# dotchen/LearningByCheating

Hardware: AMD Instinct MI355X
Metric: images/sec ImagePolicyModelSS phase-1 train @ bs256 (higher is better)
Workload: dtype bf16; 1 GPU; ImagePolicyModelSS(resnet34) phase-1 step vs BirdViewPolicyModelSS(resnet18) teacher [phase1_bs256_bf16], 160x384 RGB + 7x192x192 bird-view uint8 NHWC frames as the dataset stores them (2048-frame dataset per rank resident in HBM, a different batch every step), global batch 256 (256/GPU), bf16 MFMA operands and bf16 activation storage + f32 accumulate/master weights/gradients/BN/loss/Adam, local B; global_batch=256, parallelism=dp1

## Files before the change

### learningbycheating_amd/csrc/c_api_ops.cpp

```cpp
#include "lbc_common.hpp"
#include "lbc_hip.h"
#include "lbc_kernels.hpp"
#include <string.h>
#include <algorithm>

namespace {
size_t up64(size_t n) { return (n + 63) / 64 * 64; }
NormConst imagenet(int enabled)
{
    NormConst nc;
    memset(&nc, 0, sizeof(nc));
    nc.enabled = enabled;
    const float m3[3] = {0.485f, 0.456f, 0.406f}, s3[3] = {0.229f, 0.224f, 0.225f};
    for (int i = 0; i < 3; ++i) { nc.mean[i] = m3[i]; nc.stdv[i] = s3[i]; }
    return nc;
}
#define LBC_TRY(expr)            \
    do {                         \
        int rc__ = (expr);       \
        if (rc__) return rc__;   \
    } while (0)
}

extern "C" {

int lbc_bn_stats(const void* x, long long pixels, int C, int act_bf16, float* partial, int* rows, lbc_stream_t stream)
{
    LBC_REQUIRE(pixels > 0 && C > 0 && C % 8 == 0 && C / 4 <= 256, "bn_stats: bad shape (%lld pixels, C = %d)", pixels, C);
    if (rows) *rows = lbc_chan_reduce_rows(pixels, C);
    if (!x) return LBC_OK;
    LBC_REQUIRE(partial, "bn_stats: null partial buffer");
    ChanReduceArgs r;
    memset(&r, 0, sizeof(r));
    r.x = x; r.partial = partial; r.pixels = pixels; r.C = C; r.act_bf16 = act_bf16;
    return lbc_chan_reduce(r, 0, (hipStream_t)stream);
}

int lbc_bn_finalize_stats(const float* partial, int rows, int C, long long count, const float* gamma, const float* beta,
                          float* running_mean, float* running_var, long long* num_batches_tracked, float momentum, float eps,
                          int train, float* scale, float* shift, float* save_mean, float* save_invstd, lbc_stream_t stream)
{
    LBC_REQUIRE(scale && shift && C > 0, "bn_finalize_stats: null output");
    LBC_REQUIRE(!train || (partial && rows >= 1 && rows <= kLbcFinalizeRows && count > 0), "bn_finalize_stats: training mode needs 1..%d partial rows",
                kLbcFinalizeRows);
    LBC_REQUIRE(train || (running_mean && running_var), "bn_finalize_stats: eval mode needs the running statistics");
    LBC_REQUIRE((running_mean == nullptr) == (running_var == nullptr) && (save_mean == nullptr) == (save_invstd == nullptr),
                "bn_finalize_stats: running_mean/var and save_mean/invstd come in pairs");
    BnFinalizeArgs f;
    memset(&f, 0, sizeof(f));
    f.partial = partial; f.rows = rows; f.C = C; f.count = count; f.gamma = gamma; f.beta = beta;
    f.running_mean = running_mean; f.running_var = running_var; f.num_batches_tracked = num_batches_tracked;
    f.momentum = momentum; f.eps = eps; f.train = train;
    f.scale = scale; f.shift = shift; f.save_mean = save_mean; f.save_invstd = save_invstd;
    return lbc_bn_finalize(f, (hipStream_t)stream);
}

int lbc_bn_apply_relu_add_fwd(const void* x, void* y, long long pixels, int C, const float* scale, const float* shift,
                              const void* resid, const float* rscale, const float* rshift, int relu, int act_bf16,
                              lbc_stream_t stream)
{
    LBC_REQUIRE(x && y && scale && shift, "bn_apply: null argument");
    LBC_REQUIRE((rscale == nullptr) == (rshift == nullptr) && (!rscale || resid), "bn_apply: residual affine without a residual");
    BnApplyArgs a;
    memset(&a, 0, sizeof(a));
    a.x = x; a.y = y; a.pixels = pixels; a.C = C; a.scale = scale; a.shift = shift;
    a.resid = resid; a.rscale = rscale; a.rshift = rshift; a.relu = relu; a.act_bf16 = act_bf16;
    return lbc_bn_apply(a, (hipStream_t)stream);
}

size_t lbc_bn_bwd_workspace(int C) { return (up64((size_t)kLbcFinalizeRows * 2 * C) + 3 * up64((size_t)C)) * sizeof(float); }

int lbc_bn_bwd(const void* x, const void* dz, const void* mask, const float* mask_scale, const float* mask_shift,
               void* g_out, const float* gamma, const float* mean, const float* invstd, long long pixels, int C, int Cout,
               float* dgamma, float* dbeta, void* dx, float* workspace, int act_bf16, lbc_stream_t stream)
{
    LBC_REQUIRE(x && dz && mean && invstd && dx && workspace, "bn_bwd: null argument");
    LBC_REQUIRE(pixels > 0 && C % 8 == 0 && C / 4 <= 256 && Cout % 8 == 0 && Cout <= C, "bn_bwd: bad shape");
    LBC_REQUIRE(g_out || !mask_scale, "bn_bwd: an affine mask needs g_out (the apply pass reads the stored masked gradient)");
    hipStream_t s = (hipStream_t)stream;
    float* partial = workspace;
    float* cA = partial + up64((size_t)kLbcFinalizeRows * 2 * C);
    float* cB = cA + up64((size_t)C);
    float* cD = cB + up64((size_t)C);
    ChanReduceArgs r;
    memset(&r, 0, sizeof(r));
    r.x = x; r.dz = dz; r.mask = mask; r.mask_scale = mask_scale; r.mask_shift = mask_shift; r.g_out = g_out;
    r.mean = mean; r.invstd = invstd; r.partial = partial; r.pixels = pixels; r.C = C; r.act_bf16 = act_bf16;
    LBC_TRY(lbc_chan_reduce(r, 1, s));
    const int rows = lbc_chan_reduce_rows(pixels, C);
    BnBwdFinalizeArgs f;
    memset(&f, 0, sizeof(f));
    f.partial = partial; f.rows = rows; f.C = C; f.count = pixels; f.gamma = gamma; f.mean = mean; f.invstd = invstd; f.train = 1;
    f.dgamma = dgamma; f.dbeta = dbeta; f.coefA = cA; f.coefB = cB; f.coefD = cD;
    LBC_TRY(lbc_bn_bwd_finalize(f, s));
    BnBwdApplyArgs ap;
    memset(&ap, 0, sizeof(ap));
    ap.g = g_out ? g_out : dz; ap.mask = g_out ? nullptr : mask; ap.x = x;
    ap.coefA = cA; ap.coefB = cB; ap.coefD = cD; ap.mean = mean; ap.invstd = invstd;
    ap.dx = dx; ap.pixels = pixels; ap.C = C; ap.Cout = Cout; ap.act_bf16 = act_bf16;
    return lbc_bn_bwd_apply(ap, s);
}

int lbc_maxpool3x3s2_fwd(const void* y, const float* scale, const float* shift, void* p, unsigned char* idx, int N, int H, int W,
                         int C, int act_bf16, lbc_stream_t stream)
{
    LBC_REQUIRE(y && scale && shift && p && N > 0, "maxpool_fwd: null argument");
    PoolFwdArgs a;
    memset(&a, 0, sizeof(a));
    a.y = y; a.scale = scale; a.shift = shift; a.p = p; a.idx = idx; a.N = N; a.H = H; a.W = W; a.C = C; a.act_bf16 = act_bf16;
    return lbc_bn_relu_maxpool_fwd(a, (hipStream_t)stream);
}

int lbc_maxpool3x3s2_bwd(const void* dp, const unsigned char* idx, const void* y, const float* scale, const float* shift,
                         const float* mean, const float* invstd, void* g, float* partial, int* rows, int N, int H, int W, int C,
                         int act_bf16, lbc_stream_t stream)
{
    LBC_REQUIRE(N > 0 && H > 0 && W > 0 && C % 8 == 0 && C / 4 <= 256, "maxpool_bwd: bad shape");
    if (rows) *rows = lbc_pool_bwd_rows(N, H, W, C);
    if (!dp) return LBC_OK;
    LBC_REQUIRE(idx && y && scale && shift && mean && invstd && g && partial, "maxpool_bwd: null argument");
    PoolBwdArgs a;
    memset(&a, 0, sizeof(a));
    a.dp = dp; a.idx = idx; a.y = y; a.scale = scale; a.shift = shift; a.mean = mean; a.invstd = invstd; a.g = g; a.partial = partial;
    a.N = N; a.H = H; a.W = W; a.C = C; a.act_bf16 = act_bf16;
    return lbc_maxpool_relu_bwd_reduce(a, (hipStream_t)stream);
}

namespace {
struct HeadWs { float* rowstat; float* s_partial; float* partial2; float* coef; float* scratch; };
HeadWs head_ws(float* w, int N)
{
    HeadWs h;
    h.rowstat = w;
    h.s_partial = h.rowstat + up64((size_t)N * 40);
    h.partial2 = h.s_partial + up64((size_t)lbc_head_bwd_max_rows(N) * 20 * 65);
    h.coef = h.partial2 + up64((size_t)8 * 20 * 65);
    h.scratch = h.coef + up64((size_t)3 * 64);
    return h;
}
void head_args(const lbc_head_desc* d, HeadArgs& ha)
{
    memset(&ha, 0, sizeof(ha));
    ha.h = d->h; ha.act_bf16 = d->act_bf16; ha.N = d->N; ha.OH = d->OH; ha.OW = d->OW; ha.cmd = d->cmd;
    for (int b = 0; b < 4; ++b) {
        ha.mean[b] = d->mean[b]; ha.invstd[b] = d->invstd[b]; ha.gamma[b] = d->gamma[b]; ha.beta[b] = d->beta[b];
        ha.w[b] = d->w[b]; ha.bias[b] = d->bias[b]; ha.pos_x[b] = d->pos_x[b]; ha.pos_y[b] = d->pos_y[b];
    }
}
}

size_t lbc_head_workspace(int N)
{
    if (N < 1) return 0;
    return (up64((size_t)N * 40) + up64((size_t)lbc_head_bwd_max_rows(N) * 20 * 65) + up64((size_t)8 * 20 * 65) + up64((size_t)3 * 64) +
            up64((size_t)N * 16 * 20 * 4)) * sizeof(float);
}

int lbc_head_fwd(const lbc_head_desc* d, float* pred_all, float* pred_sel, float* workspace, lbc_stream_t stream)
{
    LBC_REQUIRE(d && d->h && d->cmd && pred_all && workspace, "head_fwd: null argument");
    HeadArgs ha;
    head_args(d, ha);
    const HeadWs ws = head_ws(workspace, d->N);
    ha.pred_all = pred_all; ha.pred_sel = pred_sel; ha.rowstat = ws.rowstat; ha.scratch = ws.scratch;
    return lbc_head_fwd(ha, (hipStream_t)stream);
}

int lbc_head_bwd(const lbc_head_desc* d, const float* pred_all, const float* d_all, const float* d_sel, void* dh,
                 float* const* dgamma, float* const* dbeta, float* const* dw, float* const* dbias, float* workspace,
                 lbc_stream_t stream)
{
    LBC_REQUIRE(d && d->h && d->cmd && pred_all && dh && dgamma && dbeta && dw && dbias && workspace, "head_bwd: null argument");
    hipStream_t s = (hipStream_t)stream;
    const int N = d->N;
    const HeadWs ws = head_ws(workspace, N);
    HeadBwdArgs hb;
    memset(&hb, 0, sizeof(hb));
    head_args(d, hb.f);
    hb.f.pred_all = const_cast<float*>(pred_all); hb.f.rowstat = ws.rowstat;
    hb.d_all = d_all; hb.d_sel = d_sel; hb.s_partial = ws.s_partial; hb.dh = dh; hb.chan_coef = ws.coef;
    LBC_TRY(lbc_head_bwd_reduce(hb, s));
    HeadBwdFinalizeArgs hf;
    memset(&hf, 0, sizeof(hf));
    hf.s_partial = ws.s_partial; hf.rows = lbc_head_bwd_rows(hb.f); hf.count = (long long)N * d->OH * d->OW;
    if (hf.rows > 8) {
        LBC_TRY(lbc_partial_reduce(ws.s_partial, hf.rows, 20 * 65, ws.partial2, 8, s));
        hf.s_partial = ws.partial2; hf.rows = 8;
    }
    for (int b = 0; b < 4; ++b) {
        hf.gamma[b] = d->gamma[b]; hf.beta[b] = d->beta[b]; hf.w[b] = d->w[b];
        hf.dgamma[b] = dgamma[b]; hf.dbeta[b] = dbeta[b]; hf.dw[b] = dw[b]; hf.dbias[b] = dbias[b];
    }
    hf.mean = d->mean[0]; hf.invstd = d->invstd[0]; hf.chan_coef = ws.coef;
    LBC_TRY(lbc_head_bwd_finalize(hf, s));
    return lbc_head_bwd_apply(hb, s);
}

int lbc_nchw_to_input(const float* image_nchw, void* xp, int xp_bf16, int N, int C, int H, int W, int normalize, lbc_stream_t stream)
{
    LBC_REQUIRE(image_nchw && xp && N > 0 && (!normalize || C == 3), "nchw_to_input: bad arguments");
    return lbc_prep_input(image_nchw, xp, xp_bf16, N, C, H, W, imagenet(normalize), (hipStream_t)stream);
}

int lbc_u8nhwc_to_input(const unsigned char* image_nhwc, void* xp, int xp_bf16, int N, int C, int H, int W, int normalize,
                        lbc_stream_t stream)
{
    LBC_REQUIRE(image_nhwc && xp && N > 0 && (!normalize || C == 3), "u8nhwc_to_input: bad arguments");
    return lbc_prep_input_u8(image_nhwc, xp, xp_bf16, N, C, H, W, imagenet(normalize), (hipStream_t)stream);
}

int lbc_stem_fwd(const void* xp, const float* w, void* y, float* stats, int* stats_rows, int N, int H, int W, int C, int bf16,
                 lbc_stream_t stream)
{
    LBC_REQUIRE(N > 0 && bf16 >= 0 && bf16 <= 2, "stem_fwd: bad arguments");
    StemArgs st;
    memset(&st, 0, sizeof(st));
    st.xp = xp; st.xp_bf16 = bf16 != 0; st.w = w; st.y = y; st.stats = stats;
    st.N = N; st.H = H; st.W = W; st.Cin = C; st.act_bf16 = bf16 == 2; st.bf16 = bf16 != 0;
    if (stats_rows) *stats_rows = lbc_stem_rows(st);
    if (!y) return LBC_OK;
    LBC_REQUIRE(xp && w, "stem_fwd: null argument");
    return lbc_stem_fwd(st, (hipStream_t)stream);
}

size_t lbc_stem_wgrad_workspace(int N, int H, int W, int C)
{
    const int ns = std::max(lbc_stem_wgrad_split(N, H, W, C, 0), lbc_stem_wgrad_split(N, H, W, C, 1));
    return (size_t)ns * 64 * 49 * C * sizeof(float);
}

int lbc_stem_wgrad(const void* xp, const void* dy, float* dw, void* workspace, int N, int H, int W, int C, int bf16,
                   lbc_stream_t stream)
{
    LBC_REQUIRE(xp && dy && dw && workspace && N > 0 && bf16 >= 0 && bf16 <= 2, "stem_wgrad: bad arguments");
    StemWgradArgs sw;
    memset(&sw, 0, sizeof(sw));
    sw.xp = xp; sw.xp_bf16 = bf16 != 0; sw.dy = dy; sw.partial = static_cast<float*>(workspace);
    sw.N = N; sw.H = H; sw.W = W; sw.Cin = C; sw.act_bf16 = bf16 == 2; sw.bf16 = bf16 != 0;
    sw.nsplit = lbc_stem_wgrad_split(N, H, W, C, bf16 != 0);
    LBC_TRY(lbc_stem_wgrad(sw, (hipStream_t)stream));
    return lbc_splitk_reduce(sw.partial, sw.nsplit, (long long)64 * 49 * C, dw, 0.f, (hipStream_t)stream);
}

int lbc_birdview_crop_u8(const unsigned char* src, unsigned char* dst, int N, int SH, int SW, int C, int y0, int x0, int H, int W,
                         lbc_stream_t stream)
{
    return lbc_crop_u8(src, dst, N, SH, SW, C, y0, x0, H, W, (hipStream_t)stream);
}

int lbc_birdview_warp_crop_u8(const unsigned char* src, unsigned char* dst, const lbc_warp_params* params_dev, int N, int SH, int SW, int C,
                              int H, int W, lbc_stream_t stream)
{
    static_assert(sizeof(lbc_warp_params) == sizeof(WarpParams), "warp parameter layout");
    return lbc_warp_crop_u8(src, dst, reinterpret_cast<const WarpParams*>(params_dev), N, SH, SW, C, H, W, (hipStream_t)stream);
}

int lbc_augment_rgb_u8(unsigned char* images, const lbc_aug_params* params_dev, float* scratch, int N, int H, int W, int any_blur,
                       lbc_stream_t stream)
{
    static_assert(sizeof(lbc_aug_params) == sizeof(AugParams), "augmentation parameter layout");
    return lbc_augment_u8(images, reinterpret_cast<const AugParams*>(params_dev), scratch, N, H, W, any_blur, (hipStream_t)stream);
}

int lbc_replay_cdf(const float* w, int n, double* cdf, long long* bad_count, lbc_stream_t stream)
{
    return lbc_replay_cdf_launch(w, n, cdf, bad_count, (hipStream_t)stream);
}

int lbc_replay_sample(const double* cdf, int n, unsigned seed, unsigned long long step, int B, int* idx, lbc_stream_t stream)
{
    return lbc_replay_sample_launch(cdf, n, seed, step, B, idx, (hipStream_t)stream);
}

int lbc_replay_gather_u8(const unsigned char* src, long long row_bytes, const int* idx, int B, int reps, unsigned char* dst, lbc_stream_t stream)
{
    return lbc_replay_gather_launch(src, row_bytes, idx, B, reps, dst, (hipStream_t)stream);
}

int lbc_replay_scatter_u8(const unsigned char* src, long long row_bytes, const int* slot, int M, unsigned char* dst, lbc_stream_t stream)
{
    return lbc_replay_scatter_launch(src, row_bytes, slot, M, dst, (hipStream_t)stream);
}

int lbc_replay_meta(const float* speed, const int* cmd, const int* idx, int B, int reps, float* speed_out, float* onehot_out, lbc_stream_t stream)
{
    return lbc_replay_meta_launch(speed, cmd, idx, B, reps, speed_out, onehot_out, (hipStream_t)stream);
}

int lbc_replay_writeback(const float* w_batch, const int* idx, int B, int reps, int n, float* new_w, lbc_stream_t stream)
{
    return lbc_replay_writeback_launch(w_batch, idx, B, reps, n, new_w, (hipStream_t)stream);
}

}
```

### learningbycheating_amd/csrc/engine.cpp

```cpp
#include "engine.hpp"

#include <algorithm>
#include <stdlib.h>
#include <string.h>

namespace lbc {

namespace {
constexpr float kBnMomentum = 0.1f;
constexpr float kBnEps = 1e-5f;
size_t up64(size_t n) { return (n + 63) / 64 * 64; }
#define LBC_TRY(expr)            \
    do {                         \
        int rc__ = (expr);       \
        if (rc__) return rc__;   \
    } while (0)
}

int Net::add_tensor(const std::string& name, int kind, std::initializer_list<int> shape)
{
    TensorInfo ti;
    ti.name = name;
    ti.kind = kind;
    ti.ndim = (int)shape.size();
    ti.numel = 1;
    int i = 0;
    for (int s : shape) { ti.shape[i++] = s; ti.numel *= s; }
    for (; i < 4; ++i) ti.shape[i] = 1;
    t_.push_back(ti);
    return (int)t_.size() - 1;
}

size_t Net::alloc(size_t nfloats)
{
    const size_t off = ws_floats_;
    ws_floats_ += up64(nfloats);
    return off;
}

size_t Net::alloc_act(size_t n) { return alloc(act_bf16_ ? (n + 1) / 2 : n); }

BN Net::make_bn(const std::string& p, int C)
{
    BN bn;
    bn.C = C;
    bn.g = add_tensor(p + ".weight", kParam, {C});
    bn.b = add_tensor(p + ".bias", kParam, {C});
    bn.rm = add_tensor(p + ".running_mean", kBufferF32, {C});
    bn.rv = add_tensor(p + ".running_var", kBufferF32, {C});
    bn.nbt = add_tensor(p + ".num_batches_tracked", kBufferI64, {});
    bn.scale = alloc(C); bn.shift = alloc(C); bn.mean = alloc(C); bn.invstd = alloc(C);
    bn.cA = alloc(C); bn.cB = alloc(C); bn.cD = alloc(C);
    return bn;
}

Conv Net::make_conv(const std::string& name, int Cin, int Cout, int H, int W, int k, int s, int p)
{
    Conv c;
    c.w = add_tensor(name, kParam, {Cout, Cin, k, k});
    c.Cin = Cin; c.Cout = Cout; c.H = H; c.W = W; c.k = k; c.s = s; c.p = p;
    c.OH = (H + 2 * p - k) / s + 1;
    c.OW = (W + 2 * p - k) / s + 1;
    c.y = alloc_act((size_t)d_.max_batch * c.OH * c.OW * Cout);
    if (act_bf16_) { c.wn = alloc(((size_t)Cout * Cin * k * k + 1) / 2); c.wt = alloc(((size_t)Cout * Cin * k * k + 1) / 2); }
    return c;
}

Net::Net(const lbc_net_desc& d) : d_(d)
{
    const size_t NB = (size_t)d.max_batch;
    const int Cin = d.in_channels, H0 = d.H, W0 = d.W;
    side_allowed_ = !lbc_opt_on(kOptNoSideStream);
    bf16_ = d.precision >= 1;
    act_bf16_ = d.precision == 2;
    x3_ = d.precision == 3;
    stem_bf16_ = bf16_ && !x3_;
    defer_wgrad_ = act_bf16_;
    if (defer_wgrad_) side_allowed_ = false;
    if (bf16_) dgrad_wt_ = true;

    stem_w_ = add_tensor("conv.conv1.weight", kParam, {64, Cin, 7, 7});
    stem_bn_ = make_bn("conv.bn1", 64);
    xp_ = alloc(NB * (H0 + 6) * (W0 + 6) * Cin);
    y0_ = alloc_act(NB * (H0 / 2) * (W0 / 2) * 64);
    H1_ = H0 / 4; W1_ = W0 / 4;
    p0_ = alloc_act(NB * H1_ * W1_ * 64);
    idx_ = alloc(NB * H1_ * W1_ * 64 / 4);

    const int n34[4] = {3, 4, 6, 3}, n18[4] = {2, 2, 2, 2};
    const int* nb = d.arch == 34 ? n34 : n18;
    int inpl = 64, h = H1_, w = W1_;
    size_t max_act = NB * H1_ * W1_ * 64;
    for (int li = 0; li < 4; ++li) {
        const int planes = 64 << li;
        stage_first_block_.push_back((int)blocks_.size());
        for (int bi = 0; bi < nb[li]; ++bi) {
            const int stride = (li > 0 && bi == 0) ? 2 : 1;
            const std::string pre = "conv.layer" + std::to_string(li + 1) + "." + std::to_string(bi);
            Block b;
            b.c1 = make_conv(pre + ".conv1.weight", inpl, planes, h, w, 3, stride, 1);
            b.b1 = make_bn(pre + ".bn1", planes);
            const int oh = b.c1.OH, ow = b.c1.OW;
            b.c2 = make_conv(pre + ".conv2.weight", planes, planes, oh, ow, 3, 1, 1);
            b.b2 = make_bn(pre + ".bn2", planes);
            if (stride != 1 || inpl != planes) {
                b.has_ds = true;
                b.ds = make_conv(pre + ".downsample.0.weight", inpl, planes, h, w, 1, stride, 0);
                b.bd = make_bn(pre + ".downsample.1", planes);
            }
            b.fuse_z1 = planes == 64 || !conv_takes_glds(b.c2, (int)NB) || conv_takes_glds(b.c2, (int)NB, true);
            b.z1 = b.fuse_z1 ? 0 : alloc_act(NB * oh * ow * planes);
            b.out = alloc_act(NB * oh * ow * planes);
            blocks_.push_back(b);
            inpl = planes; h = oh; w = ow;
        }
    }

    hcat_ = alloc_act(NB * h * w * 640);
    const int dc[4] = {640, 256, 128, 64};
    const char* bn_name[3] = {"deconv.0", "deconv.3", "deconv.6"};
    const char* ct_name[3] = {"deconv.1", "deconv.4", "deconv.7"};
    int dh = h, dw = w;
    for (int i = 0; i < 3; ++i) {
        Deconv& D = dec_[i];
        D.bn = make_bn(bn_name[i], dc[i]);
        D.w = add_tensor(std::string(ct_name[i]) + ".weight", kParam, {dc[i], dc[i + 1], 3, 3});
        D.bias = add_tensor(std::string(ct_name[i]) + ".bias", kParam, {dc[i + 1]});
        D.Cin = dc[i]; D.Cout = dc[i + 1]; D.H = dh; D.W = dw;
        D.u = alloc_act(NB * (2 * dh) * (2 * dw) * dc[i + 1]);
        if (act_bf16_) { D.wn = alloc(((size_t)dc[i] * dc[i + 1] * 9 + 1) / 2); D.wt = alloc(((size_t)dc[i] * dc[i + 1] * 9 + 1) / 2); }
        dh *= 2; dw *= 2;
        max_act = std::max(max_act, NB * dh * dw * (size_t)dc[i + 1]);
    }
    HH_ = dh; HW_ = dw;

    for (int b = 0; b < 4; ++b) {
        const std::string pre = "location_pred." + std::to_string(b);
        head_bn_[b] = make_bn(pre + ".0", 64);
        head_w_[b] = add_tensor(pre + ".1.weight", kParam, {5, 64, 1, 1});
        head_b_[b] = add_tensor(pre + ".1.bias", kParam, {5});
        head_px_[b] = add_tensor(pre + ".2.pos_x", kBufferF32, {HH_ * HW_});
        head_py_[b] = add_tensor(pre + ".2.pos_y", kBufferF32, {HH_ * HW_});
    }
    head_stats_ = alloc(2 * 64);
    head_coef_ = alloc(3 * 64);
    head_partial_ = alloc(std::max((size_t)lbc_head_bwd_max_rows((int)NB) * 20 * 65, NB * 16 * 20 * 4));
    pred_all_ = alloc(NB * 40);
    rowstat_ = alloc(NB * 40);
    cmd_ = alloc(NB * 4);

    size_t pf = 1024 * 2 * 640;
    pf = std::max(pf, (size_t)lbc_cdiv((long long)NB * (H0 / 2) * (W0 / 2), 128) * 128);
    for (const Block& b : blocks_) {
        pf = std::max(pf, (size_t)lbc_cdiv((long long)NB * b.c1.OH * b.c1.OW, 64) * 2 * b.c1.Cout);
    }
    for (int i = 0; i < 3; ++i)
        pf = std::max(pf, (size_t)4 * lbc_cdiv((long long)NB * dec_[i].H * dec_[i].W, 64) * 2 * dec_[i].Cout);
    partial_floats_ = pf;
    partial_ = alloc(pf);
    partial2_floats_ = (size_t)64 * 2 * 640;
    partial2_ = alloc(partial2_floats_);

    size_t wg = 0;
    auto wg_need = [&](int N, int OH, int OW, int CP, int Hq, int Wq, int CQ, int k, int s, int p) {
        WgradArgs a;
        memset(&a, 0, sizeof(a));
        a.N = N; a.OH = OH; a.OW = OW; a.CP = CP; a.H = Hq; a.W = Wq; a.CQ = CQ; a.KH = k; a.KW = k; a.S = s; a.P = p;
        a.bf16 = bf16_; a.act_bf16 = act_bf16_; a.x3 = x3_;
        return (size_t)lbc_wgrad_pick_split(a) * CP * k * k * CQ;
    };
    for (const Block& b : blocks_) {
        wg = std::max(wg, wg_need((int)NB, b.c1.OH, b.c1.OW, b.c1.Cout, b.c1.H, b.c1.W, b.c1.Cin, 3, b.c1.s, 1));
        wg = std::max(wg, wg_need((int)NB, b.c2.OH, b.c2.OW, b.c2.Cout, b.c2.H, b.c2.W, b.c2.Cin, 3, 1, 1));
        if (b.has_ds) wg = std::max(wg, wg_need((int)NB, b.ds.OH, b.ds.OW, b.ds.Cout, b.ds.H, b.ds.W, b.ds.Cin, 1, b.ds.s, 0));
    }
    for (int i = 0; i < 3; ++i)
        wg = std::max(wg, wg_need((int)NB, dec_[i].H, dec_[i].W, dec_[i].Cin, 2 * dec_[i].H, 2 * dec_[i].W, dec_[i].Cout, 3, 2, 1));
    wg = std::max(wg, (size_t)lbc_stem_wgrad_split((int)NB, H0, W0, Cin, stem_bf16_) * 64 * 49 * Cin);
    if (defer_wgrad_) {
        for (size_t li = 0; li < stage_first_block_.size(); ++li) {
            const size_t first = stage_first_block_[li], last = li + 1 < stage_first_block_.size() ? (size_t)stage_first_block_[li + 1] : blocks_.size();
            size_t members = 0, dy = 0;
            for (size_t bi = first; bi < last; ++bi) {
                const Block& b = blocks_[bi];
                const size_t slot = (((size_t)NB * b.c1.OH * b.c1.OW * b.c1.Cout + 1) / 2 + 63) / 64 * 64;
                members += 1 + (b.c1.s == 1 ? 1 : 0);
                dy += (b.has_ds ? 3 : 2) * slot;
            }
            const Conv& c = blocks_[last - 1].c2;
            WgradArgs a;
            memset(&a, 0, sizeof(a));
            a.N = (int)NB; a.OH = c.OH; a.OW = c.OW; a.CP = c.Cout; a.H = c.H; a.W = c.W; a.CQ = c.Cin; a.KH = 3; a.KW = 3; a.S = 1; a.P = 1;
            a.bf16 = 1; a.act_bf16 = 1; a.p = &a; a.q = &a;
            if (lbc_wgrad_tr_eligible(a)) {
                for (int n = 1; n <= (int)std::min(members, (size_t)kLbcWgradGroupMax); ++n)
                    wg = std::max(wg, (size_t)lbc_wgrad_tr_group_split(a, n) * n * c.Cout * 9 * c.Cin);
            }
            dy_arena_floats_ = std::max(dy_arena_floats_, dy);
        }
        dy_arena_ = alloc(dy_arena_floats_);
    }
    wg_partial_ = alloc(wg);
    wg_floats_ = wg;

    wt_ = alloc((size_t)640 * 512 * 9);
    gD_ = alloc_act(max_act); gE_ = alloc_act(max_act); gF_ = alloc_act(max_act); gG_ = alloc_act(max_act);
    g0_ = alloc_act(NB * (H0 / 2) * (W0 / 2) * 64);
}

std::vector<Net::ActInfo> Net::activations() const
{
    std::vector<ActInfo> v;
    const int ae = act_bf16_ ? 2 : 4;
    auto add = [&](const std::string& name, size_t off_floats, int H, int W, int C, int elem) {
        v.push_back(ActInfo{name, off_floats * sizeof(float), H, W, C, elem});
    };
    add("conv.conv1", y0_, d_.H / 2, d_.W / 2, 64, ae);
    add("conv.maxpool", p0_, H1_, W1_, 64, ae);
    add("conv.maxpool.idx", idx_, H1_, W1_, 64, 1);
    int li = 0;
    for (size_t i = 0; i < blocks_.size(); ++i) {
        while (li + 1 < (int)stage_first_block_.size() && (int)i >= stage_first_block_[li + 1]) ++li;
        const Block& b = blocks_[i];
        const std::string p = "conv.layer" + std::to_string(li + 1) + "." + std::to_string((int)i - stage_first_block_[li]);
        add(p + ".conv1", b.c1.y, b.c1.OH, b.c1.OW, b.c1.Cout, ae);
        add(p + ".bn1.scale", b.b1.scale, 1, 1, b.b1.C, 4);
        add(p + ".bn1.shift", b.b1.shift, 1, 1, b.b1.C, 4);
        add(p + ".conv2", b.c2.y, b.c2.OH, b.c2.OW, b.c2.Cout, ae);
        if (b.has_ds) add(p + ".downsample.0", b.ds.y, b.ds.OH, b.ds.OW, b.ds.Cout, ae);
        add(p, b.out, b.c2.OH, b.c2.OW, b.c2.Cout, ae);
    }
    for (int i = 0; i < 3; ++i) add("deconv." + std::to_string(3 * i + 2), dec_[i].u, 2 * dec_[i].H, 2 * dec_[i].W, dec_[i].Cout, ae);
    return v;
}

Net::~Net()
{
    if (side_) (void)hipStreamDestroy(side_);
    if (ev_fork_) (void)hipEventDestroy(ev_fork_);
    if (ev_join_) (void)hipEventDestroy(ev_join_);
}

int Net::fork(hipStream_t s)
{
    if (!side_on_) return LBC_OK;
    if (hipEventRecord(ev_fork_, s) != hipSuccess || hipStreamWaitEvent(side_, ev_fork_, 0) != hipSuccess) {
        lbc_set_error("net.backward: side-stream fork failed");
        return LBC_ELAUNCH;
    }
    side_dirty_ = true;
    return LBC_OK;
}

int Net::join(hipStream_t s)
{
    if (!side_on_ || !side_dirty_) return LBC_OK;
    if (hipEventRecord(ev_join_, side_) != hipSuccess || hipStreamWaitEvent(s, ev_join_, 0) != hipSuccess) {
        lbc_set_error("net.backward: side-stream join failed");
        return LBC_ELAUNCH;
    }
    side_dirty_ = false;
    return LBC_OK;
}

int Net::check_bound(bool need_grads) const
{
    if (!ws_) { lbc_set_error("net: workspace not bound"); return LBC_ESTATE; }
    for (const TensorInfo& t : t_) {
        if (!t.ptr) { lbc_set_error("net: tensor %s not bound", t.name.c_str()); return LBC_ESTATE; }
        if (need_grads && t.kind == kParam && !t.grad) { lbc_set_error("net: gradient of %s not bound", t.name.c_str()); return LBC_ESTATE; }
    }
    return LBC_OK;
}

int Net::conv_fwd(const Conv& c, const float* x, int N, bool stats, int* rows, hipStream_t s, const BN* pre, const BN* post,
                  const float* resid, bool relu, float* out, float* stats_buf, size_t stats_cap)
{
    IgemmArgs a;
    memset(&a, 0, sizeof(a));
    a.x = x; a.w = P(c.w); a.y = out ? out : W(c.y);
    if (pre) { a.pre_scale = W(pre->scale); a.pre_shift = W(pre->shift); a.pre_relu = 1; }
    if (post) { a.post_scale = W(post->scale); a.post_shift = W(post->shift); }
    a.resid = resid; a.relu = relu ? 1 : 0;
    a.N = N; a.H = c.H; a.W = c.W; a.C = c.Cin;
    a.OH = c.OH; a.OW = c.OW; a.K = c.Cout;
    a.KH = c.k; a.KW = c.k; a.S = c.s; a.P = c.p;
    a.M = N * c.OH * c.OW; a.LH = c.OH; a.LW = c.OW; a.ostep = 1;
    a.bf16 = bf16_; a.act_bf16 = act_bf16_; a.x3 = x3_;
    if (act_bf16_) { a.w = W(c.wn); a.w_bf16 = 1; }
    split_scratch(a);
    const int cfg = lbc_igemm_pick_for(a, 0);
    *rows = lbc_igemm_rows(a, cfg);
    a.stats = stats ? (stats_buf ? stats_buf : W(partial_)) : nullptr;
    LBC_REQUIRE(!a.stats || (size_t)*rows * 2 * (size_t)c.Cout <= (stats_buf ? stats_cap : partial_floats_),
                "net: %d statistics rows of %d channels exceed their buffer", *rows, c.Cout);
    return lbc_igemm_launch(a, 1, 0, cfg, s);
}

void Net::split_scratch(IgemmArgs& a) const
{
    if (!defer_wgrad_ || side_on_ || !wg_floats_) return;
    a.split_ws = W(wg_partial_);
    a.split_ws_floats = (long long)wg_floats_;
}

bool Net::conv_takes_glds(const Conv& c, int N, bool with_prologue) const
{
    if (!act_bf16_) return false;
    IgemmArgs a;
    memset(&a, 0, sizeof(a));
    a.N = N; a.H = c.H; a.W = c.W; a.C = c.Cin; a.OH = c.OH; a.OW = c.OW; a.K = c.Cout;
    a.KH = c.k; a.KW = c.k; a.S = c.s; a.P = c.p; a.M = N * c.OH * c.OW; a.LH = c.OH; a.LW = c.OW; a.ostep = 1;
    a.bf16 = 1; a.act_bf16 = 1; a.w_bf16 = 1;
    if (with_prologue) { a.pre_scale = reinterpret_cast<const float*>(this); a.pre_shift = a.pre_scale; a.pre_relu = 1; }
    return lbc_igemm_pick_for(a, 0) >= kLbcCfgGlds;
}

int Net::weight_prep(hipStream_t s)
{
    WeightPrepArgs a;
    memset(&a, 0, sizeof(a));
    int n = 0, tiles = 0;
    auto add = [&](const float* w, size_t wn, size_t wt, int A, int T, int B) {
        if (n >= WeightPrepArgs::kMax) return false;
        WeightPrepItem& it = a.item[n++];
        it.w = w; it.wn = W(wn); it.wt = W(wt); it.A = A; it.T = T; it.B = B; it.tile_begin = tiles;
        tiles += lbc_weight_prep_tiles(A, T, B);
        return true;
    };
    bool ok = true;
    for (const Block& b : blocks_) {
        ok = ok && add(P(b.c1.w), b.c1.wn, b.c1.wt, b.c1.Cout, 9, b.c1.Cin);
        ok = ok && add(P(b.c2.w), b.c2.wn, b.c2.wt, b.c2.Cout, 9, b.c2.Cin);
        if (b.has_ds) ok = ok && add(P(b.ds.w), b.ds.wn, b.ds.wt, b.ds.Cout, 1, b.ds.Cin);
    }
    for (int i = 0; i < 3; ++i) ok = ok && add(P(dec_[i].w), dec_[i].wn, dec_[i].wt, dec_[i].Cin, 9, dec_[i].Cout);
    LBC_REQUIRE(ok, "net: more than %d convolution weights", WeightPrepArgs::kMax);
    a.count = n; a.tiles = tiles;
    return lbc_weight_prep(a, s);
}

int Net::bn_eval_prep(hipStream_t s)
{
    BnEvalArgs a;
    memset(&a, 0, sizeof(a));
    int n = 0;
    bool ok = true;
    auto add = [&](const BN& bn) {
        if (n >= BnEvalArgs::kMax) { ok = false; return; }
        BnEvalItem& it = a.item[n++];
        it.gamma = P(bn.g); it.beta = P(bn.b); it.running_mean = P(bn.rm); it.running_var = P(bn.rv);
        it.scale = W(bn.scale); it.shift = W(bn.shift); it.mean = W(bn.mean); it.invstd = W(bn.invstd);
        it.C = bn.C;
    };
    add(stem_bn_);
    for (const Block& b : blocks_) { add(b.b1); add(b.b2); if (b.has_ds) add(b.bd); }
    for (int i = 0; i < 3; ++i) add(dec_[i].bn);
    for (int b = 0; b < 4; ++b) add(head_bn_[b]);
    LBC_REQUIRE(ok, "net: more than %d BatchNorms", BnEvalArgs::kMax);
    a.count = n; a.eps = kBnEps;
    return lbc_bn_eval_prep(a, s);
}

int Net::set_sync_bn(lbc_allreduce_fn fn, void* ctx, int world, float* buf, int buf_floats)
{
    if (!fn) { sync_fn_ = nullptr; sync_ctx_ = nullptr; sync_world_ = 1; sync_buf_ = nullptr; return LBC_OK; }
    LBC_REQUIRE(world >= 1 && buf && buf_floats >= kSyncFloats, "net.set_sync_bn: world_size >= 1 and a buffer of >= %d floats",
                kSyncFloats);
    sync_fn_ = fn; sync_ctx_ = ctx; sync_world_ = world; sync_buf_ = buf;
    return LBC_OK;
}

int Net::sync_rows(const float*& part, int& rows, int width, int n_local, hipStream_t s, float* local_lo, float* local_hi)
{
    if (!sync_fn_) return LBC_OK;
    LBC_REQUIRE(width + 1 <= kSyncFloats, "net: %d sums do not fit the SyncBN buffer", width);
    if (rows > kLbcFinalizeRows) {
        LBC_TRY(lbc_partial_reduce(part, rows, width, W(partial2_), 64, s));
        part = W(partial2_); rows = 64;
    }
    LBC_TRY(lbc_partial_reduce(part, rows, width, sync_buf_, 1, s, local_lo, local_hi, (float)n_local));
    if (sync_fn_(sync_ctx_, sync_buf_, width + 1, s) != 0) {
        lbc_set_error("net: the SyncBN all-reduce callback failed");
        return LBC_ELAUNCH;
    }
    part = sync_buf_; rows = 1;
    return LBC_OK;
}

int Net::bn_finalize(const BN& bn, int rows, long long count, int n_local, int train, hipStream_t s, bool update_running, const float* synced)
{
    const float* part = W(partial_);
    const float* nsum = nullptr;
    if (train && synced) {
        part = synced; rows = 1; nsum = synced + 2 * bn.C;
    } else if (train && sync_fn_) {
        LBC_TRY(sync_rows(part, rows, 2 * bn.C, n_local, s));
        nsum = part + 2 * bn.C;
    } else if (train && rows > kLbcFinalizeRows) {
        LBC_TRY(lbc_partial_reduce(W(partial_), rows, 2 * bn.C, W(partial2_), 64, s));
        part = W(partial2_);
        rows = 64;
    }
    BnFinalizeArgs f = fin_args(bn, part, rows, count, update_running);
    f.nsum = nsum; f.n_local = n_local; f.train = train;
    if (!train) { f.running_mean = P(bn.rm); f.running_var = P(bn.rv); f.num_batches_tracked = nullptr; }
    return lbc_bn_finalize(f, s);
}

BnFinalizeArgs Net::fin_args(const BN& bn, const float* part, int rows, long long count, bool update_running) const
{
    BnFinalizeArgs f;
    memset(&f, 0, sizeof(f));
    f.partial = part; f.rows = rows; f.C = bn.C; f.count = count;
    f.gamma = P(bn.g); f.beta = P(bn.b);
    f.running_mean = update_running ? P(bn.rm) : nullptr;
    f.running_var = update_running ? P(bn.rv) : nullptr;
    f.num_batches_tracked = update_running ? static_cast<long long*>(t_[bn.nbt].ptr) : nullptr;
    f.momentum = kBnMomentum; f.eps = kBnEps; f.train = 1;
    f.scale = W(bn.scale); f.shift = W(bn.shift); f.save_mean = W(bn.mean); f.save_invstd = W(bn.invstd);
    return f;
}

int Net::forward(int N, int train, const void* image, int image_u8, const float* velocity, const float* command, float* pred_sel,
                 float* pred_all, hipStream_t s)
{
    LBC_REQUIRE(N >= 1 && N <= d_.max_batch, "net.forward: batch %d outside [1,%d]", N, d_.max_batch);
    LBC_REQUIRE(image && velocity && command && pred_all, "net.forward: null argument");
    LBC_TRY(check_bound(false));
    lastN_ = N; last_train_ = train; ++generation_;
    const int H0 = d_.H, W0 = d_.W, Cin = d_.in_channels;
    const bool tr = train != 0;
    int rows = 0;

    LBC_TRY(lbc_copy_f32(command, W(cmd_), 4 * N, s));
    NormConst nc;
    memset(&nc, 0, sizeof(nc));
    nc.enabled = d_.normalize;
    const float m3[3] = {0.485f, 0.456f, 0.406f}, s3[3] = {0.229f, 0.224f, 0.225f};
    for (int i = 0; i < 3; ++i) { nc.mean[i] = m3[i]; nc.stdv[i] = s3[i]; }
    if (image_u8) LBC_TRY(lbc_prep_input_u8(static_cast<const unsigned char*>(image), W(xp_), stem_bf16_, N, Cin, H0, W0, nc, s));
    else          LBC_TRY(lbc_prep_input(static_cast<const float*>(image), W(xp_), stem_bf16_, N, Cin, H0, W0, nc, s));
    const bool reuse = frozen_ && derived_valid_ && !tr;
    if (act_bf16_ && !reuse) LBC_TRY(weight_prep(s));
    if (!tr && !reuse) LBC_TRY(bn_eval_prep(s));
    derived_valid_ = frozen_ && !tr;

    StemArgs st;
    st.xp = W(xp_); st.xp_bf16 = stem_bf16_; st.w = P(stem_w_); st.y = W(y0_); st.stats = tr ? W(partial_) : nullptr;
    st.N = N; st.H = H0; st.W = W0; st.Cin = Cin; st.act_bf16 = act_bf16_; st.bf16 = stem_bf16_;
    LBC_TRY(lbc_stem_fwd(st, s));
    if (tr) LBC_TRY(bn_finalize(stem_bn_, lbc_stem_rows(st), (long long)N * (H0 / 2) * (W0 / 2), N, train, s));
    PoolFwdArgs pf;
    pf.y = W(y0_); pf.scale = W(stem_bn_.scale); pf.shift = W(stem_bn_.shift); pf.p = W(p0_);
    pf.idx = reinterpret_cast<unsigned char*>(W(idx_));
    pf.N = N; pf.H = H0 / 2; pf.W = W0 / 2; pf.C = 64; pf.act_bf16 = act_bf16_;
    LBC_TRY(lbc_bn_relu_maxpool_fwd(pf, s));

    const float* x = W(p0_);
    for (Block& b : blocks_) {
        const long long pix = (long long)N * b.c1.OH * b.c1.OW;
        if (!tr) {
            LBC_TRY(conv_fwd(b.c1, x, N, false, &rows, s, nullptr, &b.b1, nullptr, true));
            const float* identity = x;
            if (b.has_ds) {
                LBC_TRY(conv_fwd(b.ds, x, N, false, &rows, s, nullptr, &b.bd, nullptr, false));
                identity = W(b.ds.y);
            }
            LBC_TRY(conv_fwd(b.c2, W(b.c1.y), N, false, &rows, s, nullptr, &b.b2, identity, true, W(b.out)));
            x = W(b.out);
            continue;
        }
        LBC_TRY(conv_fwd(b.c1, x, N, tr, &rows, s));
        const bool fold1 = !b.fuse_z1 && can_fold(rows, b.b1.C);
        if (!fold1) LBC_TRY(bn_finalize(b.b1, rows, pix, N, train, s));
        BnApplyArgs ap;
        if (b.fuse_z1) {
            LBC_TRY(conv_fwd(b.c2, W(b.c1.y), N, tr, &rows, s, &b.b1));
        } else {
            memset(&ap, 0, sizeof(ap));
            ap.x = W(b.c1.y); ap.y = W(b.z1); ap.pixels = pix; ap.C = b.c1.Cout;
            ap.scale = W(b.b1.scale); ap.shift = W(b.b1.shift); ap.relu = 1; ap.act_bf16 = act_bf16_;
            if (fold1) { ap.fold = 1; ap.fin = fin_args(b.b1, W(partial_), rows, pix); }
            LBC_TRY(lbc_bn_apply(ap, s));
            LBC_TRY(conv_fwd(b.c2, W(b.z1), N, tr, &rows, s));
        }
        const bool fold2 = can_fold(rows, b.b2.C) && (!b.has_ds || (size_t)lbc_cdiv(pix, 64) * 2 * b.bd.C <= partial2_floats_);
        const int rows2 = rows;
        if (!fold2) LBC_TRY(bn_finalize(b.b2, rows, pix, N, train, s));
        memset(&ap, 0, sizeof(ap));
        ap.x = W(b.c2.y); ap.y = W(b.out); ap.pixels = pix; ap.C = b.c2.Cout;
        ap.scale = W(b.b2.scale); ap.shift = W(b.b2.shift); ap.relu = 1; ap.act_bf16 = act_bf16_;
        if (fold2) { ap.fold = 1; ap.fin = fin_args(b.b2, W(partial_), rows2, pix); }
        if (b.has_ds) {
            float* dsp = fold2 ? W(partial2_) : W(partial_);
            LBC_TRY(conv_fwd(b.ds, x, N, tr, &rows, s, nullptr, nullptr, nullptr, false, nullptr, dsp, fold2 ? partial2_floats_ : partial_floats_));
            if (fold2 && can_fold(rows, b.bd.C)) { ap.rfold = 1; ap.rfin = fin_args(b.bd, dsp, rows, pix); }
            else if (fold2) LBC_TRY(lbc_bn_finalize(fin_args(b.bd, dsp, rows, pix), s));
            else LBC_TRY(bn_finalize(b.bd, rows, pix, N, train, s));
            ap.resid = W(b.ds.y); ap.rscale = W(b.bd.scale); ap.rshift = W(b.bd.shift);
        } else {
            ap.resid = x;
        }
        LBC_TRY(lbc_bn_apply(ap, s));
        x = W(b.out);
    }

    const Block& last = blocks_.back();
    const int th = last.c2.OH, tw = last.c2.OW;
    LBC_TRY(lbc_concat_velocity(x, velocity, W(hcat_), N, th * tw, 512, 128, act_bf16_, s));
    if (tr) {
        ChanReduceArgs cr;
        memset(&cr, 0, sizeof(cr));
        cr.x = W(hcat_); cr.partial = W(partial_); cr.pixels = (long long)N * th * tw; cr.C = 640; cr.act_bf16 = act_bf16_;
        cr.max_rows = fold_rows_for(cr.pixels, 640);
        LBC_TRY(lbc_chan_reduce(cr, 0, s));
        rows = lbc_chan_reduce_rows(cr.pixels, 640, cr.max_rows);
    }
    int pend_rows = rows;
    long long pend_count = (long long)N * th * tw;
    const float* din = W(hcat_);
    for (int i = 0; i < 3; ++i) {
        Deconv& D = dec_[i];
        IgemmArgs a;
        memset(&a, 0, sizeof(a));
        a.x = din; a.w = P(D.w); a.y = W(D.u); a.bias = P(D.bias); a.relu = 1;
        a.pre_scale = W(D.bn.scale); a.pre_shift = W(D.bn.shift);
        a.N = N; a.H = D.H; a.W = D.W; a.C = D.Cin;
        a.OH = 2 * D.H; a.OW = 2 * D.W; a.K = D.Cout;
        a.KH = 3; a.KW = 3; a.S = 2; a.P = 1;
        a.LH = D.H; a.LW = D.W; a.ostep = 2;
        a.M = N * D.H * D.W;
        a.stats = tr ? W(partial_) : nullptr;
        a.act_bf16 = act_bf16_;
        int wmajor = 0;
        if (act_bf16_) {
            a.w = W(D.wt); a.w_bf16 = 1; a.bf16 = 1; wmajor = 1;
        } else if (bf16_) {
            LBC_TRY(lbc_weight_transpose(P(D.w), W(wt_), D.Cin, 9, D.Cout, s));
            a.w = W(wt_); a.bf16 = 1; a.x3 = x3_; wmajor = 1;
        }
        a.nphase = 4;
        int cfg = lbc_igemm_pick(a.M, a.K);
        if (act_bf16_) {
            IgemmArgs b = a;
            b.pre_scale = nullptr; b.pre_shift = nullptr; b.x = W(gF_);
            const int c2 = lbc_igemm_pick_for(b, 1);
            if (c2 >= kLbcCfgGlds) {
                BnApplyArgs ap;
                memset(&ap, 0, sizeof(ap));
                ap.x = din; ap.y = W(gF_); ap.pixels = (long long)N * D.H * D.W; ap.C = D.Cin;
                ap.scale = W(D.bn.scale); ap.shift = W(D.bn.shift); ap.relu = 0; ap.act_bf16 = 1;
                if (tr && can_fold(pend_rows, D.Cin)) { ap.fold = 1; ap.fin = fin_args(D.bn, W(partial_), pend_rows, pend_count); pend_rows = 0; }
                else if (tr) { LBC_TRY(bn_finalize(D.bn, pend_rows, pend_count, N, train, s)); pend_rows = 0; }
                LBC_TRY(lbc_bn_apply(ap, s));
                a = b; cfg = c2;
            }
        }
        if (tr && pend_rows > 0) LBC_TRY(bn_finalize(D.bn, pend_rows, pend_count, N, train, s));
        const int per = lbc_igemm_rows(a, cfg);
        LBC_TRY(lbc_igemm_launch(a, wmajor, 1, cfg, s));
        const long long opix = (long long)N * 4 * D.H * D.W;
        if (!tr) {
        } else if (i < 2) {
            pend_rows = 4 * per; pend_count = opix;
        } else {
            const float* part = W(partial_);
            int prow = 4 * per;
            LBC_TRY(sync_rows(part, prow, 2 * 64, N, s));
            {
                BnFinalizeArgs f = fin_args(head_bn_[0], part, prow, opix);
                if (sync_fn_) { f.nsum = part + 2 * 64; f.n_local = N; }
                else if (prow > kLbcFinalizeRows) {
                    LBC_TRY(lbc_partial_reduce(W(partial_), prow, 2 * 64, W(partial2_), 64, s));
                    f.partial = W(partial2_); f.rows = 64;
                }
                for (int b = 1; b < 4; ++b) {
                    f.more_running_mean[b - 1] = P(head_bn_[b].rm); f.more_running_var[b - 1] = P(head_bn_[b].rv);
                    f.more_num_batches_tracked[b - 1] = static_cast<long long*>(t_[head_bn_[b].nbt].ptr);
                }
                LBC_TRY(lbc_bn_finalize(f, s));
            }
        }
        din = W(D.u);
    }

    HeadArgs ha;
    memset(&ha, 0, sizeof(ha));
    ha.h = W(dec_[2].u);
    for (int b = 0; b < 4; ++b) {
        ha.mean[b] = W(head_bn_[tr ? 0 : b].mean);
        ha.invstd[b] = W(head_bn_[tr ? 0 : b].invstd);
        ha.gamma[b] = P(head_bn_[b].g); ha.beta[b] = P(head_bn_[b].b);
        ha.w[b] = P(head_w_[b]); ha.bias[b] = P(head_b_[b]);
        ha.pos_x[b] = P(head_px_[b]); ha.pos_y[b] = P(head_py_[b]);
    }
    ha.cmd = W(cmd_);
    ha.pred_all = W(pred_all_); ha.pred_sel = pred_sel; ha.rowstat = W(rowstat_);
    ha.N = N; ha.OH = HH_; ha.OW = HW_; ha.act_bf16 = act_bf16_;
    ha.scratch = W(head_partial_);
    LBC_TRY(lbc_head_fwd(ha, s));
    return lbc_copy_f32(W(pred_all_), pred_all, 40 * N, s);
}

int Net::bn_bwd_finalize(BnBwdFinalizeArgs f, hipStream_t s)
{
    if (sync_fn_) {
        LBC_TRY(sync_rows(f.partial, f.rows, 2 * f.C, lastN_, s, f.dbeta, f.dgamma));
        f.nsum = f.partial + 2 * f.C; f.n_local = lastN_;
        f.dgamma = nullptr; f.dbeta = nullptr;
    }
    return lbc_bn_bwd_finalize(f, s);
}

int Net::bn_backward(const BN& bn, const float* dz, const float* mask, float* g_out, const float* x, long long pixels,
                     float* dx, int Cout, hipStream_t s, const BN* mask_bn, bool join_before_apply, int reduced_rows)
{
    int rows = reduced_rows;
    if (reduced_rows <= 0) {
        ChanReduceArgs r;
        memset(&r, 0, sizeof(r));
        r.x = x; r.dz = dz; r.mask = mask; r.g_out = g_out; r.mean = W(bn.mean); r.invstd = W(bn.invstd);
        if (mask_bn) { r.mask_scale = W(mask_bn->scale); r.mask_shift = W(mask_bn->shift); }
        r.partial = W(partial_); r.pixels = pixels; r.C = bn.C; r.act_bf16 = act_bf16_;
        r.max_rows = fold_rows_for(pixels, bn.C);
        LBC_TRY(lbc_chan_reduce(r, 1, s));
        rows = lbc_chan_reduce_rows(pixels, bn.C, r.max_rows);
    } else {
        mask = nullptr;
        g_out = const_cast<float*>(dz);
    }
    const float* part = W(partial_);
    if (rows > kLbcFinalizeRows) {
        LBC_TRY(lbc_partial_reduce(W(partial_), rows, 2 * bn.C, W(partial2_), 64, s));
        part = W(partial2_); rows = 64;
    }
    BnBwdFinalizeArgs f;
    memset(&f, 0, sizeof(f));
    f.partial = part; f.rows = rows; f.C = bn.C; f.count = pixels;
    f.gamma = P(bn.g); f.mean = W(bn.mean); f.invstd = W(bn.invstd); f.train = 1;
    f.dgamma = G(bn.g); f.dbeta = G(bn.b);
    f.coefA = W(bn.cA); f.coefB = W(bn.cB); f.coefD = W(bn.cD);
    const bool fold = can_fold(rows, bn.C) && (g_out || !mask);
    if (!fold) LBC_TRY(bn_bwd_finalize(f, s));
    BnBwdApplyArgs ap;
    memset(&ap, 0, sizeof(ap));
    if (fold) { ap.fold = 1; ap.fin = f; }
    ap.g = g_out ? g_out : dz; ap.mask = g_out ? nullptr : mask; ap.x = x;
    ap.coefA = W(bn.cA); ap.coefB = W(bn.cB); ap.coefD = W(bn.cD);
    ap.mean = W(bn.mean); ap.invstd = W(bn.invstd);
    ap.dx = dx; ap.pixels = pixels; ap.C = bn.C; ap.Cout = Cout; ap.act_bf16 = act_bf16_;
    if (join_before_apply) LBC_TRY(join(s));
    return lbc_bn_bwd_apply(ap, s);
}

float* Net::dy_slot(long long elems)
{
    const size_t floats = ((size_t)(elems + 1) / 2 + 63) / 64 * 64;
    if (dy_used_ + floats > dy_arena_floats_) return nullptr;
    float* p = W(dy_arena_) + dy_used_;
    dy_used_ += floats;
    return p;
}

int Net::flush_wgrads(int N, hipStream_t s)
{
    std::vector<char> done(pending_.size(), 0);
    for (size_t i = 0; i < pending_.size(); ++i) {
        if (done[i]) continue;
        const PendingWgrad& pi = pending_[i];
        const Conv& c = *pi.c;
        WgradArgs a;
        memset(&a, 0, sizeof(a));
        a.p = pi.dy; a.q = pi.x;
        if (pi.pre) { a.q_scale = W(pi.pre->scale); a.q_shift = W(pi.pre->shift); a.q_relu = 1; }
        a.bf16 = bf16_; a.act_bf16 = act_bf16_; a.x3 = x3_;
        a.N = N; a.OH = c.OH; a.OW = c.OW; a.CP = c.Cout; a.H = c.H; a.W = c.W; a.CQ = c.Cin;
        a.KH = c.k; a.KW = c.k; a.S = c.s; a.P = c.p;
        if (!lbc_wgrad_tr_eligible(a)) {
            LBC_TRY(conv_wgrad_pre(c, pi.x, pi.pre, pi.dy, N, s));
            done[i] = 1;
            continue;
        }
        WgradGroup g;
        memset(&g, 0, sizeof(g));
        float* grads[kLbcWgradGroupMax];
        for (size_t j = i; j < pending_.size() && g.n < kLbcWgradGroupMax; ++j) {
            const PendingWgrad& pj = pending_[j];
            const Conv& cj = *pj.c;
            if (done[j] || cj.Cout != c.Cout || cj.Cin != c.Cin || cj.H != c.H || cj.W != c.W || cj.k != c.k || cj.s != c.s || cj.p != c.p ||
                (pj.pre != nullptr) != (pi.pre != nullptr)) continue;
            g.p[g.n] = pj.dy; g.q[g.n] = pj.x;
            if (pj.pre) { g.q_scale[g.n] = W(pj.pre->scale); g.q_shift[g.n] = W(pj.pre->shift); }
            grads[g.n] = G(cj.w);
            ++g.n;
            done[j] = 1;
        }
        a.nsplit = lbc_wgrad_tr_group_split(a, g.n);
        const size_t count = (size_t)c.Cout * 9 * c.Cin;
        if ((size_t)a.nsplit * g.n * count > wg_floats_) a.nsplit = (int)std::max<size_t>(1, wg_floats_ / (g.n * count));
        for (int m = 0; m < g.n; ++m) g.out[m] = a.nsplit == 1 ? grads[m] : W(wg_partial_) + (size_t)m * a.nsplit * count;
        LBC_TRY(lbc_wgrad_tr_group_launch(a, g, s));
        if (a.nsplit > 1) LBC_TRY(lbc_splitk_reduce_group(W(wg_partial_), a.nsplit, (long long)count, g.n, grads, s));
    }
    pending_.clear();
    dy_used_ = 0;
    return LBC_OK;
}

int Net::conv_wgrad(const Conv& c, const float* x, const float* dy, int N, hipStream_t s)
{
    return conv_wgrad_pre(c, x, nullptr, dy, N, s);
}

int Net::conv_wgrad_pre(const Conv& c, const float* x, const BN* pre, const float* dy, int N, hipStream_t s)
{
    WgradArgs a;
    memset(&a, 0, sizeof(a));
    a.p = dy; a.q = x; a.partial = W(wg_partial_);
    if (pre) { a.q_scale = W(pre->scale); a.q_shift = W(pre->shift); a.q_relu = 1; }
    a.bf16 = bf16_; a.act_bf16 = act_bf16_; a.x3 = x3_;
    a.N = N; a.OH = c.OH; a.OW = c.OW; a.CP = c.Cout;
    a.H = c.H; a.W = c.W; a.CQ = c.Cin;
    a.KH = c.k; a.KW = c.k; a.S = c.s; a.P = c.p;
    a.nsplit = lbc_wgrad_pick_split(a);
    {
        const size_t count = (size_t)c.Cout * c.k * c.k * c.Cin;
        if ((size_t)a.nsplit * count > wg_floats_) a.nsplit = (int)std::max<size_t>(1, wg_floats_ / count);
    }
    if (a.nsplit == 1) { a.partial = G(c.w); return lbc_wgrad_launch(a, s); }
    LBC_TRY(lbc_wgrad_launch(a, s));
    return lbc_splitk_reduce(a.partial, a.nsplit, (long long)c.Cout * c.k * c.k * c.Cin, G(c.w), 0.f, s);
}

int Net::conv_dgrad(const Conv& c, const float* dy, const float* resid, float* dx, int N, hipStream_t s, const BN* bnb,
                    const float* bnb_y, int* fused_rows, const float* bnb_mask)
{
    if (fused_rows) *fused_rows = 0;
    IgemmArgs a;
    memset(&a, 0, sizeof(a));
    a.x = dy; a.w = P(c.w); a.y = dx; a.resid = resid;
    a.N = N; a.H = c.OH; a.W = c.OW; a.C = c.Cout;
    a.OH = c.H; a.OW = c.W; a.K = c.Cin;
    a.KH = c.k; a.KW = c.k; a.S = c.s; a.P = c.p;
    int wmajor = 0;
    a.bf16 = bf16_; a.act_bf16 = act_bf16_; a.x3 = x3_;
    if (act_bf16_) {
        a.w = W(c.wt); a.w_bf16 = 1; wmajor = 1;
    } else if (dgrad_wt_ && (c.k == 3 || bf16_)) {
        LBC_TRY(lbc_weight_transpose(P(c.w), W(wt_), c.Cout, c.k * c.k, c.Cin, s));
        a.w = W(wt_);
        wmajor = 1;
    }
    if (c.s == 1) {
        a.LH = c.H; a.LW = c.W; a.ostep = 1;
        a.M = N * c.H * c.W;
        split_scratch(a);
        const int cfg = wmajor ? lbc_igemm_pick_for(a, 1) : lbc_igemm_pick(a.M, a.K);
        if (bnb && bnb_y && fused_rows &&
            (bnb_mask ? lbc_igemm_fuses_bn_bwd_masked(a, wmajor, 1, cfg) : lbc_igemm_fuses_bn_bwd(a, wmajor, 1, cfg))) {
            a.bnb_y = bnb_y; a.bnb_scale = W(bnb->scale); a.bnb_shift = W(bnb->shift);
            a.bnb_mean = W(bnb->mean); a.bnb_invstd = W(bnb->invstd);
            a.bnb_mask = bnb_mask;
            a.stats = W(partial_);
            *fused_rows = lbc_igemm_rows(a, cfg);
            LBC_REQUIRE((size_t)*fused_rows * 2 * (size_t)a.K <= partial_floats_, "net: %d rows of BatchNorm-backward sums exceed their buffer", *fused_rows);
        }
        return lbc_igemm_launch(a, wmajor, 1, cfg, s);
    }
    a.LH = c.H / 2; a.LW = c.W / 2; a.ostep = 2;
    a.M = N * a.LH * a.LW;
    a.nphase = c.k == 1 ? 1 : 4;
    const int cfg = (wmajor && act_bf16_) ? lbc_igemm_pick_for(a, 1) : lbc_igemm_pick(a.M, a.K);
    return lbc_igemm_launch(a, wmajor, 1, cfg, s);
}

int Net::block_backward(Block& b, float*& D, float*& Gbuf, float* E, float* F, hipStream_t s)
{
    const int N = lastN_;
    const long long pix = (long long)N * b.c1.OH * b.c1.OW;
    const float* xin = (&b == &blocks_.front()) ? W(p0_) : W((&b - 1)->out);
    if (defer_wgrad_) {
        float* E2 = dy_slot(pix * b.b2.C);
        float* E1 = dy_slot(pix * b.b1.C);
        LBC_REQUIRE(E1 && E2, "net.backward: dY arena exhausted");
        const int pre_rows = bwd_pre_rows_;
        bwd_pre_rows_ = 0;
        LBC_REQUIRE(pre_rows == 0 || (bwd_pre_pix_ == pix && bwd_pre_C_ == b.b2.C), "net.backward: pre-reduced rows of %lld x %d do not match this block's bn2 (%lld x %d)",
                    bwd_pre_pix_, bwd_pre_C_, pix, b.b2.C);
        LBC_TRY(bn_backward(b.b2, D, W(b.out), D, W(b.c2.y), pix, E2, b.b2.C, s, nullptr, false, pre_rows));
        int fr = 0;
        LBC_TRY(conv_dgrad(b.c2, E2, nullptr, F, N, s, &b.b1, W(b.c1.y), &fr));
        if (b.fuse_z1) {
            pending_.push_back({&b.c2, W(b.c1.y), &b.b1, E2});
            LBC_TRY(bn_backward(b.b1, F, W(b.c1.y), F, W(b.c1.y), pix, E1, b.b1.C, s, &b.b1, false, fr));
        } else {
            pending_.push_back({&b.c2, W(b.z1), nullptr, E2});
            LBC_TRY(bn_backward(b.b1, F, W(b.z1), F, W(b.c1.y), pix, E1, b.b1.C, s, nullptr, false, fr));
        }
        pending_.push_back({&b.c1, xin, nullptr, E1});
        if (!b.has_ds) {
            Block* pb = (&b == &blocks_.front()) ? nullptr : (&b - 1);
            int pr = 0;
            if (pb) LBC_TRY(conv_dgrad(b.c1, E1, D, Gbuf, N, s, &pb->b2, W(pb->c2.y), &pr, W(pb->out)));
            else    LBC_TRY(conv_dgrad(b.c1, E1, D, Gbuf, N, s));
            bwd_pre_rows_ = pr;
            if (pr > 0) { bwd_pre_pix_ = (long long)N * pb->c2.OH * pb->c2.OW; bwd_pre_C_ = pb->b2.C; }
        } else {
            float* Fd = dy_slot(pix * b.bd.C);
            LBC_REQUIRE(Fd, "net.backward: dY arena exhausted");
            LBC_TRY(conv_dgrad(b.c1, E1, nullptr, Gbuf, N, s));
            LBC_TRY(bn_backward(b.bd, D, nullptr, nullptr, W(b.ds.y), pix, Fd, b.bd.C, s));
            pending_.push_back({&b.ds, xin, nullptr, Fd});
            LBC_TRY(conv_dgrad(b.ds, Fd, Gbuf, Gbuf, N, s));
        }
        std::swap(D, Gbuf);
        return LBC_OK;
    }
    LBC_TRY(bn_backward(b.b2, D, W(b.out), D, W(b.c2.y), pix, E, b.b2.C, s, nullptr, true));
    LBC_TRY(fork(s));
    int fr = 0;
    if (b.fuse_z1) {
        LBC_TRY(conv_wgrad_pre(b.c2, W(b.c1.y), &b.b1, E, N, wstream(s)));
        LBC_TRY(conv_dgrad(b.c2, E, nullptr, F, N, s, &b.b1, W(b.c1.y), &fr));
        LBC_TRY(bn_backward(b.b1, F, W(b.c1.y), F, W(b.c1.y), pix, E, b.b1.C, s, &b.b1, true, fr));
    } else {
        LBC_TRY(conv_wgrad(b.c2, W(b.z1), E, N, wstream(s)));
        LBC_TRY(conv_dgrad(b.c2, E, nullptr, F, N, s, &b.b1, W(b.c1.y), &fr));
        LBC_TRY(bn_backward(b.b1, F, W(b.z1), F, W(b.c1.y), pix, E, b.b1.C, s, nullptr, true, fr));
    }
    LBC_TRY(fork(s));
    LBC_TRY(conv_wgrad(b.c1, xin, E, N, wstream(s)));
    if (!b.has_ds) {
        LBC_TRY(conv_dgrad(b.c1, E, D, Gbuf, N, s));
    } else {
        LBC_TRY(conv_dgrad(b.c1, E, nullptr, Gbuf, N, s));
        LBC_TRY(bn_backward(b.bd, D, nullptr, nullptr, W(b.ds.y), pix, F, b.bd.C, s));
        LBC_TRY(fork(s));
        LBC_TRY(conv_wgrad(b.ds, xin, F, N, wstream(s)));
        LBC_TRY(conv_dgrad(b.ds, F, Gbuf, Gbuf, N, s));
    }
    std::swap(D, Gbuf);
    return LBC_OK;
}

int Net::backward(const float* d_sel, const float* d_all, int stage, hipStream_t s)
{
    const int rc = backward_impl(d_sel, d_all, stage, s);
    if (rc != LBC_OK) { pending_.clear(); dy_used_ = 0; bwd_pre_rows_ = 0; }
    if (rc != LBC_OK && side_dirty_) {
        (void)hipStreamSynchronize(side_);
        side_dirty_ = false;
    }
    return rc;
}

int Net::backward_impl(const float* d_sel, const float* d_all, int stage, hipStream_t s)
{
    LBC_REQUIRE(lastN_ > 0 && last_train_, "net.backward: needs a preceding training-mode forward");
    LBC_REQUIRE(stage >= -1 && stage < kNumStages, "net.backward: bad stage %d", stage);
    LBC_TRY(check_bound(true));
    const int N = lastN_;
    float* E = W(gE_);
    float* F = W(gF_);
    side_on_ = side_allowed_ && !lbc_prof_on();
    if (side_on_ && !side_) {
        int cur = 0, want = 0;
        (void)hipGetDevice(&cur);
        want = cur;
        hipPointerAttribute_t attr;
        if (hipPointerGetAttributes(&attr, ws_) == hipSuccess) want = attr.device;
        if (want != cur) (void)hipSetDevice(want);
        const bool ok = hipStreamCreateWithFlags(&side_, hipStreamNonBlocking) == hipSuccess &&
                        hipEventCreateWithFlags(&ev_fork_, hipEventDisableTiming) == hipSuccess &&
                        hipEventCreateWithFlags(&ev_join_, hipEventDisableTiming) == hipSuccess;
        if (want != cur) (void)hipSetDevice(cur);
        if (!ok) {
            lbc_set_error("net.backward: cannot create the side stream");
            return LBC_ELAUNCH;
        }
    }

    if (stage == -1 || stage == 0) {
        bwd_D_ = W(gD_); bwd_G_ = W(gG_);
        HeadBwdArgs hb;
        memset(&hb, 0, sizeof(hb));
        HeadArgs& ha = hb.f;
        ha.h = W(dec_[2].u);
        for (int b = 0; b < 4; ++b) {
            ha.mean[b] = W(head_bn_[0].mean); ha.invstd[b] = W(head_bn_[0].invstd);
            ha.gamma[b] = P(head_bn_[b].g); ha.beta[b] = P(head_bn_[b].b);
            ha.w[b] = P(head_w_[b]); ha.bias[b] = P(head_b_[b]);
            ha.pos_x[b] = P(head_px_[b]); ha.pos_y[b] = P(head_py_[b]);
        }
        ha.cmd = W(cmd_); ha.pred_all = W(pred_all_); ha.rowstat = W(rowstat_);
        ha.N = N; ha.OH = HH_; ha.OW = HW_; ha.act_bf16 = act_bf16_;
        hb.d_all = d_all; hb.d_sel = d_sel; hb.s_partial = W(head_partial_); hb.dh = E; hb.chan_coef = W(head_coef_);
        LBC_TRY(lbc_head_bwd_reduce(hb, s));
        HeadBwdFinalizeArgs hf;
        memset(&hf, 0, sizeof(hf));
        hf.s_partial = W(head_partial_); hf.rows = lbc_head_bwd_rows(hb.f); hf.count = (long long)N * HH_ * HW_;
        if (hf.rows > 8) {
            LBC_TRY(lbc_partial_reduce(W(head_partial_), hf.rows, 20 * 65, W(partial2_), 8, s));
            hf.s_partial = W(partial2_); hf.rows = 8;
        }
        for (int b = 0; b < 4; ++b) {
            hf.gamma[b] = P(head_bn_[b].g); hf.beta[b] = P(head_bn_[b].b); hf.w[b] = P(head_w_[b]);
            hf.dgamma[b] = G(head_bn_[b].g); hf.dbeta[b] = G(head_bn_[b].b);
            hf.dw[b] = G(head_w_[b]); hf.dbias[b] = G(head_b_[b]);
        }
        hf.mean = W(head_bn_[0].mean); hf.invstd = W(head_bn_[0].invstd); hf.chan_coef = W(head_coef_);
        LBC_TRY(lbc_head_bwd_finalize(hf, s));
        if (sync_fn_) {
            LBC_TRY(sync_rows(hf.s_partial, hf.rows, 20 * 65, N, s));
            hf.nsum = hf.s_partial + 20 * 65; hf.n_local = N; hf.coef_only = 1;
            LBC_TRY(lbc_head_bwd_finalize(hf, s));
        }
        LBC_TRY(lbc_head_bwd_apply(hb, s));

        for (int i = 2; i >= 0; --i) {
            Deconv& D = dec_[i];
            const float* xin = i == 0 ? W(hcat_) : W(dec_[i - 1].u);
            const long long opix = (long long)N * 4 * D.H * D.W;
            const long long ipix = (long long)N * D.H * D.W;
            ChanReduceArgs r;
            memset(&r, 0, sizeof(r));
            r.dz = E; r.mask = W(D.u); r.g_out = E; r.partial = W(partial_); r.pixels = opix; r.C = D.Cout; r.act_bf16 = act_bf16_;
            LBC_TRY(lbc_chan_reduce(r, 1, s));
            int rows = lbc_chan_reduce_rows(opix, D.Cout);
            const float* part = W(partial_);
            if (rows > kLbcFinalizeRows) {
                LBC_TRY(lbc_partial_reduce(W(partial_), rows, 2 * D.Cout, W(partial2_), 64, s));
                part = W(partial2_); rows = 64;
            }
            BnBwdFinalizeArgs f;
            memset(&f, 0, sizeof(f));
            f.partial = part; f.rows = rows; f.C = D.Cout; f.count = opix; f.dbeta = G(D.bias);
            LBC_TRY(lbc_bn_bwd_finalize(f, s));
            WgradArgs wa;
            memset(&wa, 0, sizeof(wa));
            wa.p = xin; wa.q = E; wa.partial = W(wg_partial_);
            wa.p_scale = W(D.bn.scale); wa.p_shift = W(D.bn.shift);
            wa.N = N; wa.OH = D.H; wa.OW = D.W; wa.CP = D.Cin;
            wa.H = 2 * D.H; wa.W = 2 * D.W; wa.CQ = D.Cout; wa.KH = 3; wa.KW = 3; wa.S = 2; wa.P = 1;
            wa.bf16 = bf16_; wa.act_bf16 = act_bf16_; wa.x3 = x3_;
            wa.nsplit = lbc_wgrad_pick_split(wa);
            if ((size_t)wa.nsplit * D.Cin * 9 * D.Cout > wg_floats_) wa.nsplit = (int)std::max<size_t>(1, wg_floats_ / ((size_t)D.Cin * 9 * D.Cout));
            if (wa.nsplit == 1) wa.partial = G(D.w);
            LBC_TRY(lbc_wgrad_launch(wa, s));
            if (wa.nsplit > 1) LBC_TRY(lbc_splitk_reduce(wa.partial, wa.nsplit, (long long)D.Cin * 9 * D.Cout, G(D.w), 0.f, s));
            IgemmArgs a;
            memset(&a, 0, sizeof(a));
            a.x = E; a.w = P(D.w); a.y = F;
            a.N = N; a.H = 2 * D.H; a.W = 2 * D.W; a.C = D.Cout;
            a.OH = D.H; a.OW = D.W; a.K = D.Cin; a.KH = 3; a.KW = 3; a.S = 2; a.P = 1;
            a.M = N * D.H * D.W; a.LH = D.H; a.LW = D.W; a.ostep = 1;
            a.bf16 = bf16_; a.act_bf16 = act_bf16_; a.x3 = x3_;
            if (act_bf16_) { a.w = W(D.wn); a.w_bf16 = 1; }
            LBC_TRY(lbc_igemm_launch(a, 1, 0, act_bf16_ ? lbc_igemm_pick_for(a, 0) : lbc_igemm_pick(a.M, a.K), s));
            float* dst = i == 0 ? bwd_D_ : E;
            LBC_TRY(bn_backward(D.bn, F, nullptr, nullptr, xin, ipix, dst, i == 0 ? 512 : D.Cin, s));
        }
    }

    for (int li = 3; li >= 0; --li) {
        const int st = 4 - li;
        if (stage != -1 && stage != st) continue;
        bwd_pre_rows_ = 0;
        const int first = stage_first_block_[li];
        const int lastb = li == 3 ? (int)blocks_.size() : stage_first_block_[li + 1];
        for (int bi = lastb - 1; bi >= first; --bi) LBC_TRY(block_backward(blocks_[bi], bwd_D_, bwd_G_, E, F, s));
        if (defer_wgrad_) LBC_TRY(flush_wgrads(N, s));
        LBC_TRY(join(s));
    }

    if (stage == -1 || stage == 5) {
        const int H0 = d_.H, W0 = d_.W;
        PoolBwdArgs pb;
        memset(&pb, 0, sizeof(pb));
        pb.dp = bwd_D_; pb.idx = reinterpret_cast<const unsigned char*>(W(idx_)); pb.y = W(y0_);
        pb.scale = W(stem_bn_.scale); pb.shift = W(stem_bn_.shift);
        pb.mean = W(stem_bn_.mean); pb.invstd = W(stem_bn_.invstd);
        pb.g = W(g0_); pb.partial = W(partial_);
        pb.N = N; pb.H = H0 / 2; pb.W = W0 / 2; pb.C = 64; pb.act_bf16 = act_bf16_;
        LBC_TRY(lbc_maxpool_relu_bwd_reduce(pb, s));
        int rows = lbc_pool_bwd_rows(N, H0 / 2, W0 / 2, 64);
        const long long pix = (long long)N * (H0 / 2) * (W0 / 2);
        const float* part = W(partial_);
        if (rows > kLbcFinalizeRows) {
            LBC_TRY(lbc_partial_reduce(W(partial_), rows, 128, W(partial2_), 64, s));
            part = W(partial2_); rows = 64;
        }
        BnBwdFinalizeArgs f;
        memset(&f, 0, sizeof(f));
        f.partial = part; f.rows = rows; f.C = 64; f.count = pix;
        f.gamma = P(stem_bn_.g); f.mean = W(stem_bn_.mean); f.invstd = W(stem_bn_.invstd); f.train = 1;
        f.dgamma = G(stem_bn_.g); f.dbeta = G(stem_bn_.b);
        f.coefA = W(stem_bn_.cA); f.coefB = W(stem_bn_.cB); f.coefD = W(stem_bn_.cD);
        LBC_TRY(bn_bwd_finalize(f, s));
        StemWgradArgs sw;
        memset(&sw, 0, sizeof(sw));
        if (lbc_stem_wgrad_fuses_bn_bwd(d_.in_channels, stem_bf16_)) {
            sw.bn_y = W(y0_); sw.bn_coefA = W(stem_bn_.cA); sw.bn_coefB = W(stem_bn_.cB); sw.bn_coefD = W(stem_bn_.cD);
            sw.bn_mean = W(stem_bn_.mean); sw.bn_invstd = W(stem_bn_.invstd);
        } else {
            BnBwdApplyArgs ap;
            memset(&ap, 0, sizeof(ap));
            ap.g = W(g0_); ap.x = W(y0_); ap.coefA = W(stem_bn_.cA); ap.coefB = W(stem_bn_.cB); ap.coefD = W(stem_bn_.cD);
            ap.mean = W(stem_bn_.mean); ap.invstd = W(stem_bn_.invstd);
            ap.dx = W(g0_); ap.pixels = pix; ap.C = 64; ap.Cout = 64; ap.act_bf16 = act_bf16_;
            LBC_TRY(lbc_bn_bwd_apply(ap, s));
        }
        sw.xp = W(xp_); sw.xp_bf16 = stem_bf16_; sw.dy = W(g0_); sw.partial = W(wg_partial_);
        sw.N = N; sw.H = H0; sw.W = W0; sw.Cin = d_.in_channels; sw.act_bf16 = act_bf16_; sw.bf16 = stem_bf16_;
        sw.nsplit = lbc_stem_wgrad_split(N, H0, W0, d_.in_channels, stem_bf16_);
        LBC_TRY(lbc_stem_wgrad(sw, s));
        LBC_TRY(lbc_splitk_reduce(sw.partial, sw.nsplit, (long long)64 * 49 * d_.in_channels, G(stem_w_), 0.f, s));
    }
    return LBC_OK;
}

}

struct lbc_net { lbc::Net impl; explicit lbc_net(const lbc_net_desc& d) : impl(d) {} };

extern "C" {

int lbc_net_create(const lbc_net_desc* d, lbc_net** out)
{
    LBC_REQUIRE(d && out, "net_create: null argument");
    LBC_REQUIRE(d->arch == 18 || d->arch == 34, "net_create: arch %d unsupported (BasicBlock ResNet-18/34 only)", d->arch);
    LBC_REQUIRE(d->in_channels == 3 || d->in_channels == 7, "net_create: in_channels %d unsupported", d->in_channels);
    LBC_REQUIRE(d->H > 0 && d->W > 0 && d->H % 32 == 0 && d->W % 32 == 0, "net_create: image %dx%d must be a multiple of 32", d->H, d->W);
    LBC_REQUIRE(d->max_batch >= 1, "net_create: max_batch %d", d->max_batch);
    LBC_REQUIRE(!d->normalize || d->in_channels == 3, "net_create: ImageNet normalisation needs 3 channels");
    LBC_REQUIRE(d->precision >= 0 && d->precision <= 3,
                "net_create: precision %d unknown (0 = f32, 1 = bf16 MFMA operands, 2 = bf16 operands + bf16 activation storage, "
                "3 = split-bf16 operands (bf16x3))", d->precision);
    LBC_REQUIRE((long long)d->max_batch * (d->H / 2) * (d->W / 2) * 64 < (1ll << 31), "net_create: batch too large for 32-bit indexing");
    *out = new lbc_net(*d);
    return LBC_OK;
}
void lbc_net_destroy(lbc_net* net) { delete net; }
int lbc_net_num_tensors(const lbc_net* net) { return net ? (int)const_cast<lbc_net*>(net)->impl.tensors().size() : 0; }
int lbc_net_tensor_info(const lbc_net* net, int i, char* name, int name_cap, int* kind, int* ndim, int* shape4)
{
    LBC_REQUIRE(net, "tensor_info: null net");
    auto& ts = const_cast<lbc_net*>(net)->impl.tensors();
    LBC_REQUIRE(i >= 0 && i < (int)ts.size(), "tensor_info: index %d out of range", i);
    const lbc::TensorInfo& t = ts[(size_t)i];
    if (name && name_cap > 0) { strncpy(name, t.name.c_str(), (size_t)name_cap - 1); name[name_cap - 1] = 0; }
    if (kind) *kind = t.kind;
    if (ndim) *ndim = t.ndim;
    if (shape4) for (int k = 0; k < 4; ++k) shape4[k] = t.shape[k];
    return LBC_OK;
}
size_t lbc_net_workspace_bytes(const lbc_net* net) { return net ? net->impl.workspace_bytes() : 0; }
int lbc_net_num_activations(const lbc_net* net) { return net ? (int)net->impl.activations().size() : 0; }
int lbc_net_activation_info(const lbc_net* net, int i, char* name, int name_cap, size_t* offset_bytes, int* hwc3, int* elem_bytes)
{
    LBC_REQUIRE(net, "activation_info: null net");
    const auto acts = net->impl.activations();
    LBC_REQUIRE(i >= 0 && i < (int)acts.size(), "activation_info: index %d out of range", i);
    const auto& a = acts[(size_t)i];
    if (name && name_cap > 0) { strncpy(name, a.name.c_str(), (size_t)name_cap - 1); name[name_cap - 1] = 0; }
    if (offset_bytes) *offset_bytes = a.offset_bytes;
    if (hwc3) { hwc3[0] = a.H; hwc3[1] = a.W; hwc3[2] = a.C; }
    if (elem_bytes) *elem_bytes = a.elem;
    return LBC_OK;
}
int lbc_net_bind(lbc_net* net, void* workspace, void* const* tensor_ptrs, float* const* grad_ptrs)
{
    LBC_REQUIRE(net && workspace && tensor_ptrs, "net_bind: null argument");
    net->impl.set_workspace(workspace);
    net->impl.invalidate_derived();
    auto& ts = net->impl.tensors();
    for (size_t i = 0; i < ts.size(); ++i) {
        ts[i].ptr = tensor_ptrs[i];
        ts[i].grad = (grad_ptrs && ts[i].kind == lbc::kParam) ? grad_ptrs[i] : nullptr;
    }
    return LBC_OK;
}
int lbc_net_forward(lbc_net* net, int N, int train, const float* image, const float* velocity, const float* command,
                    float* pred_sel, float* pred_all, lbc_stream_t stream)
{
    LBC_REQUIRE(net, "net_forward: null net");
    return net->impl.forward(N, train, image, 0, velocity, command, pred_sel, pred_all, (hipStream_t)stream);
}
int lbc_net_forward_u8(lbc_net* net, int N, int train, const unsigned char* image_nhwc, const float* velocity, const float* command,
                       float* pred_sel, float* pred_all, lbc_stream_t stream)
{
    LBC_REQUIRE(net, "net_forward_u8: null net");
    return net->impl.forward(N, train, image_nhwc, 1, velocity, command, pred_sel, pred_all, (hipStream_t)stream);
}
int lbc_net_num_stages(void) { return lbc::Net::kNumStages; }
int lbc_net_last_forward(const lbc_net* net, int* batch, int* train, long long* generation)
{
    LBC_REQUIRE(net, "net_last_forward: null net");
    if (batch) *batch = net->impl.last_batch();
    if (train) *train = net->impl.last_train();
    if (generation) *generation = net->impl.generation();
    return LBC_OK;
}
int lbc_net_set_frozen(lbc_net* net, int frozen)
{
    LBC_REQUIRE(net, "net_set_frozen: null net");
    net->impl.set_frozen(frozen != 0);
    return LBC_OK;
}
int lbc_net_set_sync_bn(lbc_net* net, lbc_allreduce_fn fn, void* ctx, int world_size, float* buf, int buf_floats)
{
    LBC_REQUIRE(net, "net_set_sync_bn: null net");
    return net->impl.set_sync_bn(fn, ctx, world_size, buf, buf_floats);
}
int lbc_net_backward(lbc_net* net, const float* d_sel, const float* d_all, int stage, lbc_stream_t stream)
{
    LBC_REQUIRE(net, "net_backward: null net");
    return net->impl.backward(d_sel, d_all, stage, (hipStream_t)stream);
}

int lbc_loss(int kind, const lbc_camera* cam, const float* pred, const float* target, int N, int rows, float grad_scale,
             float* loss_per_sample, float* dpred, lbc_stream_t stream)
{
    LBC_REQUIRE(pred && target && loss_per_sample, "loss: null argument");
    LossArgs a;
    memset(&a, 0, sizeof(a));
    a.pred = pred; a.target = target; a.loss_per_sample = loss_per_sample; a.dpred = dpred;
    a.N = N; a.R = rows; a.grad_scale = grad_scale;
    if (cam) {
        a.w = cam->w; a.h = cam->h; a.fov = cam->fov; a.world_y = cam->world_y; a.fixed_offset = cam->fixed_offset;
        a.pixels_per_meter = cam->pixels_per_meter; a.crop_size = cam->crop_size;
    }
    if (kind == 1) { LBC_REQUIRE(cam, "loss: phase-1 needs a camera"); return lbc_loss_phase1(a, (hipStream_t)stream); }
    if (kind == 0) { LBC_REQUIRE(cam, "loss: phase-0 needs a camera"); return lbc_loss_phase0(a, (hipStream_t)stream); }
    if (kind == 2) {
        LBC_REQUIRE(cam, "loss: bird-view L1 needs crop_size");
        return lbc_loss_l1(a, 1.f / (0.5f * cam->crop_size), -1.f, (hipStream_t)stream);
    }
    if (kind == 3) return lbc_loss_l1(a, 1.f, 0.f, (hipStream_t)stream);
    lbc_set_error("loss: unknown kind %d", kind);
    return LBC_EINVAL;
}

int lbc_phase2_weight(const lbc_camera* cam, const float* pred_sel, const float* teacher_sel, int N, float* weights,
                      lbc_stream_t stream)
{
    LBC_REQUIRE(cam && pred_sel && teacher_sel && weights, "phase2_weight: null argument");
    LossArgs a;
    memset(&a, 0, sizeof(a));
    a.pred = pred_sel; a.target = teacher_sel; a.loss_per_sample = weights; a.N = N; a.R = 5;
    a.w = cam->w; a.h = cam->h; a.fov = cam->fov; a.world_y = cam->world_y; a.fixed_offset = cam->fixed_offset;
    a.pixels_per_meter = cam->pixels_per_meter; a.crop_size = cam->crop_size;
    return lbc_phase2_weight_launch(a, (hipStream_t)stream);
}

int lbc_adam_step(const lbc_adam_chunk* chunks_dev, int nchunks, double lr, double beta1, double beta2,
                  double eps, double weight_decay, int step, lbc_stream_t stream)
{
    static_assert(sizeof(lbc_adam_chunk) == sizeof(AdamChunk), "chunk layout");
    return lbc_adam_launch(reinterpret_cast<const AdamChunk*>(chunks_dev), nchunks, lr, beta1, beta2, eps, weight_decay,
                           step, (hipStream_t)stream);
}

}
```

### learningbycheating_amd/csrc/engine.hpp

```cpp
#pragma once
#include <string>
#include <vector>

#include "lbc_common.hpp"
#include "lbc_hip.h"
#include "lbc_kernels.hpp"

namespace lbc {

enum TensorKind { kParam = 0, kBufferF32 = 1, kBufferI64 = 2 };

struct TensorInfo {
    std::string name;
    int kind;
    int ndim;
    int shape[4];
    long long numel;
    void* ptr = nullptr;
    float* grad = nullptr;
};

struct BN {
    int C = 0;
    int g = -1, b = -1, rm = -1, rv = -1, nbt = -1;
    size_t scale = 0, shift = 0, mean = 0, invstd = 0;
    size_t cA = 0, cB = 0, cD = 0;
};

struct Conv {
    int w = -1;
    int Cin = 0, Cout = 0, H = 0, W = 0, k = 0, s = 1, p = 0, OH = 0, OW = 0;
    size_t y = 0;
    size_t wn = 0, wt = 0;
};

struct Block {
    Conv c1, c2, ds;
    BN b1, b2, bd;
    bool has_ds = false;
    bool fuse_z1 = true;
    size_t z1 = 0, out = 0;
};

struct Deconv {
    BN bn;
    int w = -1, bias = -1;
    int Cin = 0, Cout = 0, H = 0, W = 0;
    size_t u = 0;
    size_t wn = 0, wt = 0;
};

class Net {
public:
    explicit Net(const lbc_net_desc& d);
    ~Net();
    const lbc_net_desc& desc() const { return d_; }
    std::vector<TensorInfo>& tensors() { return t_; }
    size_t workspace_bytes() const { return ws_floats_ * sizeof(float); }
    void set_workspace(void* p) { ws_ = static_cast<float*>(p); }
    int check_bound(bool need_grads) const;

    int forward(int N, int train, const void* image, int image_u8, const float* velocity, const float* command, float* pred_sel,
                float* pred_all, hipStream_t s);
    int backward(const float* d_sel, const float* d_all, int stage, hipStream_t s);
    static const int kNumStages = 6;
    struct ActInfo { std::string name; size_t offset_bytes; int H, W, C, elem; };
    std::vector<ActInfo> activations() const;
    void set_frozen(bool f) { frozen_ = f; derived_valid_ = false; }
    void invalidate_derived() { derived_valid_ = false; }
    int last_batch() const { return lastN_; }
    int last_train() const { return last_train_; }
    long long generation() const { return generation_; }
    static const int kSyncFloats = 1536;
    int set_sync_bn(lbc_allreduce_fn fn, void* ctx, int world, float* buf, int buf_floats);

private:
    int add_tensor(const std::string& name, int kind, std::initializer_list<int> shape);
    size_t alloc(size_t nfloats);
    size_t alloc_act(size_t nelems);
    BN make_bn(const std::string& prefix, int C);
    Conv make_conv(const std::string& name, int Cin, int Cout, int H, int W, int k, int s, int p);
    float* W(size_t off) const { return ws_ + off; }
    float* P(int ti) const { return static_cast<float*>(t_[ti].ptr); }
    float* G(int ti) const { return t_[ti].grad; }

    int conv_fwd(const Conv& c, const float* x, int N, bool stats, int* rows, hipStream_t s, const BN* pre = nullptr,
                 const BN* post = nullptr, const float* resid = nullptr, bool relu = false, float* out = nullptr, float* stats_buf = nullptr,
                 size_t stats_cap = 0);
    BnFinalizeArgs fin_args(const BN& bn, const float* part, int rows, long long count, bool update_running = true) const;
    bool can_fold(int rows, int C) const { return !sync_fn_ && rows <= kLbcFinalizeRows && lbc_bn_fold_ok(rows, C); }
    int fold_rows_for(long long pixels, int C) const
    {
        if (sync_fn_ || pixels * C * (act_bf16_ ? 2 : 4) > (8ll << 20)) return 0;
        return lbc_bn_fold_ok(1, C) ? lbc_bn_fold_max_rows(C) : 0;
    }
    int bn_eval_prep(hipStream_t s);
    int conv_wgrad_pre(const Conv& c, const float* x, const BN* pre, const float* dy, int N, hipStream_t s);
    bool dgrad_wt_ = false;
    size_t wt_ = 0;
    bool bf16_ = false;
    bool act_bf16_ = false;
    bool x3_ = false;
    bool stem_bf16_ = false;
    int weight_prep(hipStream_t s);
    bool conv_takes_glds(const Conv& c, int N, bool with_prologue = false) const;
    int bn_finalize(const BN& bn, int rows, long long count, int n_local, int train, hipStream_t s, bool update_running = true,
                    const float* synced = nullptr);
    int sync_rows(const float*& part, int& rows, int width, int n_local, hipStream_t s, float* local_lo = nullptr, float* local_hi = nullptr);
    int bn_bwd_finalize(BnBwdFinalizeArgs f, hipStream_t s);
    lbc_allreduce_fn sync_fn_ = nullptr;
    void* sync_ctx_ = nullptr;
    int sync_world_ = 1;
    float* sync_buf_ = nullptr;
    int bn_backward(const BN& bn, const float* dz, const float* mask, float* g_out, const float* x, long long pixels,
                    float* dx, int Cout, hipStream_t s, const BN* mask_bn = nullptr, bool join_before_apply = false, int reduced_rows = 0);
    int fork(hipStream_t s);
    int join(hipStream_t s);
    hipStream_t wstream(hipStream_t s) const { return side_on_ ? side_ : s; }
    void split_scratch(IgemmArgs& a) const;
    hipStream_t side_ = nullptr;
    hipEvent_t ev_fork_ = nullptr, ev_join_ = nullptr;
    bool side_allowed_ = true, side_on_ = false, side_dirty_ = false;
    int conv_wgrad(const Conv& c, const float* x, const float* dy, int N, hipStream_t s);
    int conv_dgrad(const Conv& c, const float* dy, const float* resid, float* dx, int N, hipStream_t s, const BN* bnb = nullptr,
                   const float* bnb_y = nullptr, int* fused_rows = nullptr, const float* bnb_mask = nullptr);
    int block_backward(Block& b, float*& D, float*& Gbuf, float* E, float* F, hipStream_t s);
    struct PendingWgrad { const Conv* c; const float* x; const BN* pre; const float* dy; };
    std::vector<PendingWgrad> pending_;
    bool defer_wgrad_ = false;
    size_t dy_arena_ = 0, dy_arena_floats_ = 0, dy_used_ = 0;
    size_t wg_floats_ = 0;
    float* dy_slot(long long elems);
    int flush_wgrads(int N, hipStream_t s);
    int backward_impl(const float* d_sel, const float* d_all, int stage, hipStream_t s);
    long long generation_ = 0;

    lbc_net_desc d_;
    std::vector<TensorInfo> t_;
    size_t ws_floats_ = 0;
    float* ws_ = nullptr;

    int stem_w_ = -1;
    BN stem_bn_;
    int H1_ = 0, W1_ = 0;
    std::vector<Block> blocks_;
    std::vector<int> stage_first_block_;
    Deconv dec_[3];
    BN head_bn_[4];
    int head_w_[4], head_b_[4], head_px_[4], head_py_[4];
    int HH_ = 0, HW_ = 0;

    size_t xp_ = 0, y0_ = 0, p0_ = 0, idx_ = 0, hcat_ = 0, cmd_ = 0;
    size_t partial_ = 0, partial2_ = 0, wg_partial_ = 0, head_partial_ = 0, head_coef_ = 0, head_stats_ = 0;
    size_t pred_all_ = 0, rowstat_ = 0;
    size_t gD_ = 0, gE_ = 0, gF_ = 0, gG_ = 0, g0_ = 0;
    size_t partial_floats_ = 0, partial2_floats_ = 0;

    bool frozen_ = false, derived_valid_ = false;
    int lastN_ = 0;
    int last_train_ = 0;
    float* bwd_D_ = nullptr;
    long long bwd_pre_pix_ = 0; int bwd_pre_C_ = 0;
    int bwd_pre_rows_ = 0;
    float* bwd_G_ = nullptr;
};

}
```

### learningbycheating_amd/csrc/head.hip

```cpp
#include "lbc_common.hpp"
#include "lbc_act.hpp"
#include "lbc_kernels.hpp"
#include <stdlib.h>

namespace {

constexpr int TP = 256;
constexpr int LDH = 68;

struct SoftAcc { float m, l, sx, sy; };

__device__ __forceinline__ void soft_merge(SoftAcc& a, const SoftAcc& b)
{
    const float M = fmaxf(a.m, b.m);
    if (M == -INFINITY) return;
    const float fa = __expf(a.m - M), fb = __expf(b.m - M);
    a.l = a.l * fa + b.l * fb;
    a.sx = a.sx * fa + b.sx * fb;
    a.sy = a.sy * fa + b.sy * fb;
    a.m = M;
}

template <typename T>
__device__ __forceinline__ void load_tile(const void* hv, float* sH, int n, int HW, int tile, int tid)
{
    const T* h = static_cast<const T*>(hv);
#pragma unroll
    for (int j = 0; j < 16; ++j) {
        const int idx = tid + 256 * j;
        const int row = idx >> 4, sg = idx & 15;
        const int p = tile * TP + row;
        f32x4 v = {0.f, 0.f, 0.f, 0.f};
        if (p < HW) v = Act<T>::ld4(h + ((size_t)n * HW + (size_t)p) * 64 + (size_t)(sg * 4));
        *reinterpret_cast<f32x4*>(&sH[row * LDH + sg * 4]) = v;
    }
}

__device__ __forceinline__ void fold_branch(const HeadArgs& a, int b, float* sW , float* sB , int tid, int nthr)
{
    const float* mean = a.mean[b];
    const float* inv = a.invstd[b];
    for (int idx = tid; idx < 320; idx += nthr) {
        const int c = idx & 63;
        const float wf = a.w[b][idx] * a.gamma[b][c] * inv[c];
        float v = wf;
        if (a.act_bf16) {
            const float hi = (float)(__bf16)wf;
            v = a.wsplit ? hi + (float)(__bf16)(wf - hi) : hi;
        }
        sW[idx] = v;
    }
    if (tid < 5) {
        float t = a.bias[b][tid];
        for (int c = 0; c < 64; ++c)
            t += a.w[b][tid * 64 + c] * (a.beta[b][c] - a.gamma[b][c] * mean[c] * inv[c]);
        sB[tid] = t;
    }
}

template <typename T>
__global__ __launch_bounds__(256) void head_fwd_k(HeadArgs a)
{
    __shared__ __attribute__((aligned(16))) float sH[TP * LDH];
    __shared__ __attribute__((aligned(16))) float sW[320];
    __shared__ float sB[8];
    __shared__ float sRed[4 * 5 * 4];
    const int tid = threadIdx.x, lane = tid & 63, wave = tid >> 6;
    const int n = blockIdx.x, b = blockIdx.y;
    const int HW = a.OH * a.OW;
    fold_branch(a, b, sW, sB, tid, 256);
    __syncthreads();

    SoftAcc st[5];
#pragma unroll
    for (int s = 0; s < 5; ++s) { st[s].m = -INFINITY; st[s].l = 0.f; st[s].sx = 0.f; st[s].sy = 0.f; }

    const int ntile = (HW + TP - 1) / TP;
    for (int tile = 0; tile < ntile; ++tile) {
        load_tile<T>(a.h, sH, n, HW, tile, tid);
        __syncthreads();
        const int p = tile * TP + tid;
        if (p < HW) {
            float lg[5];
#pragma unroll
            for (int s = 0; s < 5; ++s) lg[s] = sB[s];
#pragma unroll
            for (int c4 = 0; c4 < 16; ++c4) {
                const float4 f = *reinterpret_cast<const float4*>(&sH[tid * LDH + c4 * 4]);
#pragma unroll
                for (int s = 0; s < 5; ++s) {
                    const float4 w = *reinterpret_cast<const float4*>(&sW[s * 64 + c4 * 4]);
                    lg[s] += f.x * w.x + f.y * w.y + f.z * w.z + f.w * w.w;
                }
            }
            const float px = a.pos_x[b][p], py = a.pos_y[b][p];
#pragma unroll
            for (int s = 0; s < 5; ++s) {
                SoftAcc o; o.m = lg[s]; o.l = 1.f; o.sx = px; o.sy = py;
                soft_merge(st[s], o);
            }
        }
        __syncthreads();
    }
#pragma unroll
    for (int s = 0; s < 5; ++s) {
#pragma unroll
        for (int off = 32; off >= 1; off >>= 1) {
            SoftAcc o;
            o.m = __shfl_xor(st[s].m, off); o.l = __shfl_xor(st[s].l, off);
            o.sx = __shfl_xor(st[s].sx, off); o.sy = __shfl_xor(st[s].sy, off);
            soft_merge(st[s], o);
        }
        if (lane == 0) {
            sRed[(wave * 5 + s) * 4 + 0] = st[s].m; sRed[(wave * 5 + s) * 4 + 1] = st[s].l;
            sRed[(wave * 5 + s) * 4 + 2] = st[s].sx; sRed[(wave * 5 + s) * 4 + 3] = st[s].sy;
        }
    }
    __syncthreads();
    if (tid < 5) {
        SoftAcc t; t.m = sRed[tid * 4]; t.l = sRed[tid * 4 + 1]; t.sx = sRed[tid * 4 + 2]; t.sy = sRed[tid * 4 + 3];
        for (int w = 1; w < 4; ++w) {
            SoftAcc o; o.m = sRed[(w * 5 + tid) * 4]; o.l = sRed[(w * 5 + tid) * 4 + 1];
            o.sx = sRed[(w * 5 + tid) * 4 + 2]; o.sy = sRed[(w * 5 + tid) * 4 + 3];
            soft_merge(t, o);
        }
        const size_t o2 = (((size_t)n * 4 + b) * 5 + tid) * 2;
        a.pred_all[o2] = t.sx / t.l;
        a.pred_all[o2 + 1] = t.sy / t.l;
        if (a.rowstat) { a.rowstat[o2] = t.m; a.rowstat[o2 + 1] = t.l; }
    }
}

__global__ __launch_bounds__(256) void head_fwd_mfma_k(HeadArgs a)
{
    __shared__ float sWf[4 * 320];
    __shared__ float sBf[4 * 8];
    __shared__ float sRed[4 * 32 * 4];
    const int tid = threadIdx.x, lane = tid & 63, wave = tid >> 6;
    const int l31 = lane & 31, kh = lane >> 5;
    const int n = blockIdx.x;
    const int HW = a.OH * a.OW;
    const int S = a.nslice, slice = blockIdx.y;
    for (int b = 0; b < 4; ++b) fold_branch(a, b, sWf + b * 320, sBf + b * 8, tid, 256);
    __syncthreads();
    const bool colok = l31 < 20;
    const int cb = colok ? l31 / 5 : 0, cs = colok ? l31 - 5 * cb : 0;
    bf16x8 wb[4], wl[4];
#pragma unroll
    for (int g = 0; g < 4; ++g)
#pragma unroll
        for (int j = 0; j < 8; ++j) {
            const float v = colok ? sWf[cb * 320 + cs * 64 + g * 16 + kh * 8 + j] : 0.f;
            wb[g][j] = (__bf16)v;
            wl[g][j] = (__bf16)(v - (float)wb[g][j]);
        }
    const bool split = a.wsplit != 0;
    const float bias = colok ? sBf[cb * 8 + cs] : 0.f;
    const float* posx = a.pos_x[cb];
    const float* posy = a.pos_y[cb];
    const __bf16* h = static_cast<const __bf16*>(a.h) + (size_t)n * HW * 64;

    SoftAcc st; st.m = -INFINITY; st.l = 0.f; st.sx = 0.f; st.sy = 0.f;
    const int ngroup = (HW + 31) / 32;
    for (int grp = slice * 4 + wave; grp < ngroup; grp += 4 * S) {
        const int pbase = grp * 32;
        const int pl = pbase + l31 < HW ? pbase + l31 : HW - 1;
        f32x16 acc;
#pragma unroll
        for (int e = 0; e < 16; ++e) acc[e] = 0.f;
        bf16x8 af[4];
#pragma unroll
        for (int g = 0; g < 4; ++g) af[g] = *reinterpret_cast<const bf16x8*>(h + (size_t)pl * 64 + (size_t)(g * 16 + kh * 8));
#pragma unroll
        for (int g = 0; g < 4; ++g) acc = __builtin_amdgcn_mfma_f32_32x32x16_bf16(af[g], wb[g], acc, 0, 0, 0);
        if (split) {
#pragma unroll
            for (int g = 0; g < 4; ++g) acc = __builtin_amdgcn_mfma_f32_32x32x16_bf16(af[g], wl[g], acc, 0, 0, 0);
        }
        float mx = -INFINITY;
#pragma unroll
        for (int e = 0; e < 16; ++e) {
            const int p = pbase + (e & 3) + 8 * (e >> 2) + 4 * kh;
            acc[e] = (p < HW && colok) ? acc[e] + bias : -INFINITY;
            mx = fmaxf(mx, acc[e]);
        }
        if (mx != -INFINITY) {
            const float M = fmaxf(st.m, mx);
            const float f = __expf(st.m - M);
            st.l *= f; st.sx *= f; st.sy *= f; st.m = M;
#pragma unroll
            for (int e = 0; e < 16; ++e) {
                const int p = pbase + (e & 3) + 8 * (e >> 2) + 4 * kh;
                const int pc = p < HW ? p : HW - 1;
                const float w = __expf(acc[e] - M);
                st.l += w; st.sx += w * posx[pc]; st.sy += w * posy[pc];
            }
        }
    }
    {
        SoftAcc o;
        o.m = __shfl_xor(st.m, 32); o.l = __shfl_xor(st.l, 32); o.sx = __shfl_xor(st.sx, 32); o.sy = __shfl_xor(st.sy, 32);
        soft_merge(st, o);
    }
    if (kh == 0) {
        sRed[(wave * 32 + l31) * 4 + 0] = st.m; sRed[(wave * 32 + l31) * 4 + 1] = st.l;
        sRed[(wave * 32 + l31) * 4 + 2] = st.sx; sRed[(wave * 32 + l31) * 4 + 3] = st.sy;
    }
    __syncthreads();
    if (tid < 20) {
        SoftAcc t; t.m = sRed[tid * 4]; t.l = sRed[tid * 4 + 1]; t.sx = sRed[tid * 4 + 2]; t.sy = sRed[tid * 4 + 3];
        for (int w = 1; w < 4; ++w) {
            SoftAcc o; o.m = sRed[(w * 32 + tid) * 4]; o.l = sRed[(w * 32 + tid) * 4 + 1];
            o.sx = sRed[(w * 32 + tid) * 4 + 2]; o.sy = sRed[(w * 32 + tid) * 4 + 3];
            soft_merge(t, o);
        }
        if (S > 1) {
            float* dst = a.scratch + (((size_t)n * S + slice) * 20 + tid) * 4;
            dst[0] = t.m; dst[1] = t.l; dst[2] = t.sx; dst[3] = t.sy;
        } else {
            const size_t o2 = ((size_t)n * 20 + tid) * 2;
            a.pred_all[o2] = t.sx / t.l;
            a.pred_all[o2 + 1] = t.sy / t.l;
            if (a.rowstat) { a.rowstat[o2] = t.m; a.rowstat[o2 + 1] = t.l; }
        }
    }
}

__global__ __launch_bounds__(256) void head_merge_k(HeadArgs a)
{
    const int i = blockIdx.x * 256 + threadIdx.x;
    if (i >= a.N * 20) return;
    const int n = i / 20, col = i - n * 20;
    const float* src = a.scratch + ((size_t)n * a.nslice * 20 + col) * 4;
    SoftAcc t; t.m = src[0]; t.l = src[1]; t.sx = src[2]; t.sy = src[3];
    for (int k = 1; k < a.nslice; ++k) {
        const float* p = src + (size_t)k * 80;
        SoftAcc o; o.m = p[0]; o.l = p[1]; o.sx = p[2]; o.sy = p[3];
        soft_merge(t, o);
    }
    a.pred_all[(size_t)i * 2] = t.sx / t.l;
    a.pred_all[(size_t)i * 2 + 1] = t.sy / t.l;
    if (a.rowstat) { a.rowstat[(size_t)i * 2] = t.m; a.rowstat[(size_t)i * 2 + 1] = t.l; }
}

__global__ __launch_bounds__(256) void select_branch_k(const float* __restrict__ all, const float* __restrict__ cmd,
                                                       float* __restrict__ sel, int N)
{
    const int i = blockIdx.x * 256 + threadIdx.x;
    if (i >= N * 10) return;
    const int n = i / 10, r = i - n * 10;
    float t = 0.f;
    for (int b = 0; b < 4; ++b) t += cmd[n * 4 + b] * all[(n * 4 + b) * 10 + r];
    sel[i] = t;
}

__device__ __forceinline__ void row_grad(const HeadBwdArgs& a, int n, int b, int s, float& gx, float& gy)
{
    gx = 0.f; gy = 0.f;
    if (a.d_all) { gx = a.d_all[((n * 4 + b) * 5 + s) * 2]; gy = a.d_all[((n * 4 + b) * 5 + s) * 2 + 1]; }
    if (a.d_sel) {
        const float cm = a.f.cmd[n * 4 + b];
        gx += cm * a.d_sel[(n * 5 + s) * 2]; gy += cm * a.d_sel[(n * 5 + s) * 2 + 1];
    }
}

template <typename T>
__global__ __launch_bounds__(256) void head_bwd_reduce_k(HeadBwdArgs a)
{
    __shared__ __attribute__((aligned(16))) float sH[TP * LDH];
    __shared__ __attribute__((aligned(16))) float sW[320];
    __shared__ float sB[8];
    __shared__ float sRow[5 * 5];
    __shared__ float sD[5 * TP];
    __shared__ float sAcc[4 * 5 * 64];
    __shared__ float sS0[4 * 5];
    const int tid = threadIdx.x, lane = tid & 63, wave = tid >> 6;
    const int n = blockIdx.x, b = blockIdx.y;
    const int HW = a.f.OH * a.f.OW;
    fold_branch(a.f, b, sW, sB, tid, 256);
    if (tid < 5) {
        float gx, gy;
        row_grad(a, n, b, tid, gx, gy);
        const size_t o2 = (((size_t)n * 4 + b) * 5 + tid) * 2;
        sRow[tid * 5 + 0] = gx; sRow[tid * 5 + 1] = gy;
        sRow[tid * 5 + 2] = gx * a.f.pred_all[o2] + gy * a.f.pred_all[o2 + 1];
        sRow[tid * 5 + 3] = a.f.rowstat[o2];
        sRow[tid * 5 + 4] = 1.f / a.f.rowstat[o2 + 1];
    }
    __syncthreads();

    const int c = tid & 63, q = tid >> 6;
    float acc[5], s0[5];
#pragma unroll
    for (int s = 0; s < 5; ++s) { acc[s] = 0.f; s0[s] = 0.f; }

    const int ntile = (HW + TP - 1) / TP;
    for (int tile = 0; tile < ntile; ++tile) {
        load_tile<T>(a.f.h, sH, n, HW, tile, tid);
        __syncthreads();
        const int p = tile * TP + tid;
        float dl[5];
#pragma unroll
        for (int s = 0; s < 5; ++s) dl[s] = 0.f;
        if (p < HW) {
            float lg[5];
#pragma unroll
            for (int s = 0; s < 5; ++s) lg[s] = sB[s];
#pragma unroll
            for (int c4 = 0; c4 < 16; ++c4) {
                const float4 f = *reinterpret_cast<const float4*>(&sH[tid * LDH + c4 * 4]);
#pragma unroll
                for (int s = 0; s < 5; ++s) {
                    const float4 w = *reinterpret_cast<const float4*>(&sW[s * 64 + c4 * 4]);
                    lg[s] += f.x * w.x + f.y * w.y + f.z * w.z + f.w * w.w;
                }
            }
            const float px = a.f.pos_x[b][p], py = a.f.pos_y[b][p];
#pragma unroll
            for (int s = 0; s < 5; ++s) {
                const float pr = __expf(lg[s] - sRow[s * 5 + 3]) * sRow[s * 5 + 4];
                dl[s] = pr * ((sRow[s * 5 + 0] * px + sRow[s * 5 + 1] * py) - sRow[s * 5 + 2]);
                s0[s] += dl[s];
            }
        }
#pragma unroll
        for (int s = 0; s < 5; ++s) sD[s * TP + tid] = dl[s];
        __syncthreads();
        for (int pp = q * 64; pp < q * 64 + 64; ++pp) {
            const float hv = sH[pp * LDH + c];
#pragma unroll
            for (int s = 0; s < 5; ++s) acc[s] += sD[s * TP + pp] * hv;
        }
        __syncthreads();
    }
#pragma unroll
    for (int s = 0; s < 5; ++s) {
        sAcc[(q * 5 + s) * 64 + c] = acc[s];
        float t = s0[s];
#pragma unroll
        for (int off = 32; off >= 1; off >>= 1) t += __shfl_xor(t, off);
        if (lane == 0) sS0[wave * 5 + s] = t;
    }
    __syncthreads();
    float* out = a.s_partial + (size_t)n * (20 * 65) + (size_t)(b * 5) * 65;
    for (int idx = tid; idx < 320; idx += 256) {
        const int s = idx >> 6, cc = idx & 63;
        out[s * 65 + cc] = sAcc[(0 * 5 + s) * 64 + cc] + sAcc[(1 * 5 + s) * 64 + cc] + sAcc[(2 * 5 + s) * 64 + cc] +
                           sAcc[(3 * 5 + s) * 64 + cc];
    }
    if (tid < 5) out[tid * 65 + 64] = sS0[tid] + sS0[5 + tid] + sS0[10 + tid] + sS0[15 + tid];
}

__global__ __launch_bounds__(256) void head_bwd_finalize_k(HeadBwdFinalizeArgs a)
{
    __shared__ float sS[20 * 65];
    __shared__ float sDG[4 * 64], sDB[4 * 64];
    const int tid = threadIdx.x;
    for (int idx = tid; idx < 20 * 65; idx += 256) {
        double t = 0.0;
        for (int r = 0; r < a.rows; ++r) t += (double)a.s_partial[(size_t)r * (20 * 65) + idx];
        sS[idx] = (float)t;
    }
    __syncthreads();
    for (int idx = tid; idx < 20 * 64; idx += 256) {
        const int bs = idx >> 6, c = idx & 63;
        const float s0 = sS[bs * 65 + 64];
        sS[bs * 65 + c] = a.invstd[c] * (sS[bs * 65 + c] - a.mean[c] * s0);
    }
    __syncthreads();
    for (int idx = tid; idx < 20 * 64; idx += 256) {
        const int bs = idx >> 6, c = idx & 63, b = bs / 5;
        if (!a.coef_only) a.dw[b][(bs - b * 5) * 64 + c] = a.gamma[b][c] * sS[bs * 65 + c] + a.beta[b][c] * sS[bs * 65 + 64];
    }
    if (tid < 20 && !a.coef_only) a.dbias[tid / 5][tid % 5] = sS[tid * 65 + 64];
    {
        const int b = tid >> 6, c = tid & 63;
        float dg = 0.f, db = 0.f;
        for (int s = 0; s < 5; ++s) {
            const float w = a.w[b][s * 64 + c];
            dg += w * sS[(b * 5 + s) * 65 + c];
            db += w * sS[(b * 5 + s) * 65 + 64];
        }
        if (!a.coef_only) { a.dgamma[b][c] = dg; a.dbeta[b][c] = db; }
        sDG[tid] = dg; sDB[tid] = db;
    }
    __syncthreads();
    if (tid < 64) {
        double k1 = 0.0, k2 = 0.0;
        for (int b = 0; b < 4; ++b) {
            k1 += (double)a.gamma[b][tid] * (double)sDB[b * 64 + tid];
            k2 += (double)a.gamma[b][tid] * (double)sDG[b * 64 + tid];
        }
        const double n = a.nsum ? (double)a.count / (double)a.n_local * (double)*a.nsum : (double)a.count;
        k1 /= n; k2 /= n;
        const double inv = (double)a.invstd[tid];
        a.chan_coef[tid] = (float)(inv * k1);
        a.chan_coef[64 + tid] = (float)(inv * k2);
    }
}

template <typename T>
__global__ __launch_bounds__(256) void head_bwd_apply_k(HeadBwdArgs a)
{
    __shared__ __attribute__((aligned(16))) float sH[TP * LDH];
    __shared__ __attribute__((aligned(16))) float sW[20 * 64];
    __shared__ float sB[4 * 8];
    __shared__ float sRow[20 * 5];
    __shared__ float sD[20 * TP];
    const int tid = threadIdx.x;
    const int n = blockIdx.x, tile = blockIdx.y;
    const int HW = a.f.OH * a.f.OW;
    for (int b = 0; b < 4; ++b) fold_branch(a.f, b, sW + b * 320, sB + b * 8, tid, 256);
    if (tid < 20) {
        const int b = tid / 5, s = tid - b * 5;
        float gx, gy;
        row_grad(a, n, b, s, gx, gy);
        const size_t o2 = (((size_t)n * 4 + b) * 5 + s) * 2;
        sRow[tid * 5 + 0] = gx; sRow[tid * 5 + 1] = gy;
        sRow[tid * 5 + 2] = gx * a.f.pred_all[o2] + gy * a.f.pred_all[o2 + 1];
        sRow[tid * 5 + 3] = a.f.rowstat[o2];
        sRow[tid * 5 + 4] = 1.f / a.f.rowstat[o2 + 1];
    }
    load_tile<T>(a.f.h, sH, n, HW, tile, tid);
    __syncthreads();
    const int p = tile * TP + tid;
    {
        float lg[20];
#pragma unroll
        for (int bs = 0; bs < 20; ++bs) lg[bs] = sB[(bs / 5) * 8 + (bs % 5)];
        if (p < HW) {
#pragma unroll
            for (int c4 = 0; c4 < 16; ++c4) {
                const float4 f = *reinterpret_cast<const float4*>(&sH[tid * LDH + c4 * 4]);
#pragma unroll
                for (int bs = 0; bs < 20; ++bs) {
                    const float4 w = *reinterpret_cast<const float4*>(&sW[bs * 64 + c4 * 4]);
                    lg[bs] += f.x * w.x + f.y * w.y + f.z * w.z + f.w * w.w;
                }
            }
        }
#pragma unroll
        for (int bs = 0; bs < 20; ++bs) {
            float d = 0.f;
            if (p < HW) {
                const int b = bs / 5;
                const float px = a.f.pos_x[b][p], py = a.f.pos_y[b][p];
                const float pr = __expf(lg[bs] - sRow[bs * 5 + 3]) * sRow[bs * 5 + 4];
                d = pr * ((sRow[bs * 5 + 0] * px + sRow[bs * 5 + 1] * py) - sRow[bs * 5 + 2]);
            }
            sD[bs * TP + tid] = d;
        }
    }
    __syncthreads();
    const int c = tid & 63, q = tid >> 6;
    float wf[20];
#pragma unroll
    for (int bs = 0; bs < 20; ++bs) wf[bs] = sW[bs * 64 + c];
    const float c1 = a.chan_coef[c], c2 = a.chan_coef[64 + c];
    const float mu = a.f.mean[0][c], iv = a.f.invstd[0][c];
    for (int pp = q * 64; pp < q * 64 + 64; ++pp) {
        const int pg = tile * TP + pp;
        if (pg >= HW) break;
        float o = -c1 - c2 * ((sH[pp * LDH + c] - mu) * iv);
#pragma unroll
        for (int bs = 0; bs < 20; ++bs) o += sD[bs * TP + pp] * wf[bs];
        Act<T>::st1(static_cast<T*>(a.dh) + ((size_t)n * HW + (size_t)pg) * 64 + c, o);
    }
}


constexpr int kHTS = 80;

struct HeadRowConst { float k0, gx, gy, cst; };

__device__ __forceinline__ void head_row_consts(const HeadBwdArgs& a, int n, const float* sBf, float* sRow , int tid)
{
    if (tid < 20) {
        const int b = tid / 5, st = tid - b * 5;
        float gx, gy;
        row_grad(a, n, b, st, gx, gy);
        const size_t o2 = (((size_t)n * 4 + b) * 5 + st) * 2;
        sRow[tid * 4 + 0] = sBf[b * 8 + st] - a.f.rowstat[o2] - logf(a.f.rowstat[o2 + 1]);
        sRow[tid * 4 + 1] = gx;
        sRow[tid * 4 + 2] = gy;
        sRow[tid * 4 + 3] = gx * a.f.pred_all[o2] + gy * a.f.pred_all[o2 + 1];
    }
}

__global__ __launch_bounds__(256, 2) void head_bwd_reduce_mfma_k(HeadBwdArgs a, int S)
{
    __shared__ float sWf[4 * 320];
    __shared__ float sBf[4 * 8];
    __shared__ float sRow[20 * 4];
    __shared__ __attribute__((aligned(16))) __bf16 sT[4][32 * kHTS];
    __shared__ float sRed[4][20 * 65];
    __shared__ float sDiff[4][20];
    const int tid = threadIdx.x, lane = tid & 63, wave = tid >> 6;
    const int l31 = lane & 31, kh = lane >> 5, G1 = (lane >> 4) & 1, t16 = lane & 15;
    const int n = blockIdx.x, slice = blockIdx.y;
    const int HW = a.f.OH * a.f.OW;
    for (int b = 0; b < 4; ++b) fold_branch(a.f, b, sWf + b * 320, sBf + b * 8, tid, 256);
    __syncthreads();
    head_row_consts(a, n, sBf, sRow, tid);
    __syncthreads();
    const bool colok = l31 < 20;
    const int cb = colok ? l31 / 5 : 0, cs = colok ? l31 - 5 * cb : 0;
    bf16x8 wb[4], wl[4];
#pragma unroll
    for (int g = 0; g < 4; ++g)
#pragma unroll
        for (int j = 0; j < 8; ++j) {
            const float v = colok ? sWf[cb * 320 + cs * 64 + g * 16 + kh * 8 + j] : 0.f;
            wb[g][j] = (__bf16)v;
            wl[g][j] = (__bf16)(v - (float)wb[g][j]);
        }
    const bool split = a.f.wsplit != 0;
    const float k0 = colok ? sRow[l31 * 4 + 0] : 0.f, gx = colok ? sRow[l31 * 4 + 1] : 0.f;
    const float gy = colok ? sRow[l31 * 4 + 2] : 0.f, cst = colok ? sRow[l31 * 4 + 3] : 0.f;
    const float* posx = a.f.pos_x[cb];
    const float* posy = a.f.pos_y[cb];
    const __bf16* h = static_cast<const __bf16*>(a.f.h) + (size_t)n * HW * 64;
    __bf16* tile = sT[wave];

    f32x16 accH[2];
#pragma unroll
    for (int c = 0; c < 2; ++c)
#pragma unroll
        for (int e = 0; e < 16; ++e) accH[c][e] = 0.f;
    float s0 = 0.f, s0r = 0.f;
    const int ngroup = (HW + 31) / 32;
    for (int grp = slice * 4 + wave; grp < ngroup; grp += 4 * S) {
        const int pbase = grp * 32;
        const int pl = pbase + l31 < HW ? pbase + l31 : HW - 1;
        bf16x8 af[4];
#pragma unroll
        for (int g = 0; g < 4; ++g) af[g] = *reinterpret_cast<const bf16x8*>(h + (size_t)pl * 64 + (size_t)(g * 16 + kh * 8));
#pragma unroll
        for (int g = 0; g < 4; ++g) *reinterpret_cast<bf16x8*>(&tile[l31 * kHTS + g * 16 + kh * 8]) = af[g];
        f32x16 acc;
#pragma unroll
        for (int e = 0; e < 16; ++e) acc[e] = 0.f;
#pragma unroll
        for (int g = 0; g < 4; ++g) acc = __builtin_amdgcn_mfma_f32_32x32x16_bf16(af[g], wb[g], acc, 0, 0, 0);
        if (split) {
#pragma unroll
            for (int g = 0; g < 4; ++g) acc = __builtin_amdgcn_mfma_f32_32x32x16_bf16(af[g], wl[g], acc, 0, 0, 0);
        }
        bf16x8 db[2];
#pragma unroll
        for (int e = 0; e < 16; ++e) {
            const int p = pbase + (e & 3) + 8 * (e >> 2) + 4 * kh;
            float d = 0.f;
            if (p < HW && colok) d = __expf(acc[e] + k0) * ((gx * posx[p] + gy * posy[p]) - cst);
            const __bf16 dr = (__bf16)d;
            db[e >> 3][e & 7] = dr;
            s0 += d;
            s0r += (float)dr;
        }
#pragma unroll
        for (int c = 0; c < 2; ++c)
#pragma unroll
            for (int j = 0; j < 2; ++j) {
                const int row = 16 * j + 4 * kh + (t16 >> 2);
                const int col = 32 * c + 16 * G1 + (t16 & 3) * 4;
                const bf16x4 a0 = lds_read_tr16(&tile[row * kHTS + col]);
                const bf16x4 a1 = lds_read_tr16(&tile[(row + 8) * kHTS + col]);
                const bf16x8 at = {a0[0], a0[1], a0[2], a0[3], a1[0], a1[1], a1[2], a1[3]};
                accH[c] = __builtin_amdgcn_mfma_f32_32x32x16_bf16(at, db[j], accH[c], 0, 0, 0);
            }
    }
    s0 += __shfl_xor(s0, 32);
    s0r += __shfl_xor(s0r, 32);
    if (colok) {
#pragma unroll
        for (int c = 0; c < 2; ++c)
#pragma unroll
            for (int e = 0; e < 16; ++e) sRed[wave][l31 * 65 + 32 * c + (e & 3) + 8 * (e >> 2) + 4 * kh] = accH[c][e];
        if (kh == 0) { sRed[wave][l31 * 65 + 64] = s0; sDiff[wave][l31] = s0r - s0; }
    }
    __syncthreads();
    float* out = a.s_partial + ((size_t)n * S + slice) * (20 * 65);
    for (int idx = tid; idx < 20 * 65; idx += 256) {
        const int bs = idx / 65, c = idx - bs * 65;
        float v = (sRed[0][idx] + sRed[1][idx]) + (sRed[2][idx] + sRed[3][idx]);
        if (c < 64) v -= a.f.mean[0][c] * ((sDiff[0][bs] + sDiff[1][bs]) + (sDiff[2][bs] + sDiff[3][bs]));
        out[idx] = v;
    }
}

__global__ __launch_bounds__(256, 2) void head_bwd_apply_mfma_k(HeadBwdArgs a, int S)
{
    __shared__ float sWf[4 * 320];
    __shared__ float sBf[4 * 8];
    __shared__ float sRow[20 * 4];
    const int tid = threadIdx.x, lane = tid & 63, wave = tid >> 6;
    const int l31 = lane & 31, kh = lane >> 5;
    const int n = blockIdx.x, slice = blockIdx.y;
    const int HW = a.f.OH * a.f.OW;
    for (int b = 0; b < 4; ++b) fold_branch(a.f, b, sWf + b * 320, sBf + b * 8, tid, 256);
    __syncthreads();
    head_row_consts(a, n, sBf, sRow, tid);
    __syncthreads();
    const bool rowok = l31 < 20;
    const int rb = rowok ? l31 / 5 : 0, rs = rowok ? l31 - 5 * rb : 0;
    bf16x8 wa[4], wal[4];
#pragma unroll
    for (int g = 0; g < 4; ++g)
#pragma unroll
        for (int j = 0; j < 8; ++j) {
            const float v = rowok ? sWf[rb * 320 + rs * 64 + g * 16 + kh * 8 + j] : 0.f;
            wa[g][j] = (__bf16)v;
            wal[g][j] = (__bf16)(v - (float)wa[g][j]);
        }
    const bool split = a.f.wsplit != 0;
    float ck0[12], cgx[12], cgy[12], ccst[12];
    int ebr[12];
#pragma unroll
    for (int e = 0; e < 12; ++e) {
        const int bs = (e & 3) + 8 * (e >> 2) + 4 * kh;
        const bool ok = bs < 20;
        ebr[e] = ok ? bs / 5 : 0;
        ck0[e] = ok ? sRow[bs * 4 + 0] : -INFINITY;
        cgx[e] = ok ? sRow[bs * 4 + 1] : 0.f;
        cgy[e] = ok ? sRow[bs * 4 + 2] : 0.f;
        ccst[e] = ok ? sRow[bs * 4 + 3] : 0.f;
    }
    bf16x8 wt[2][2], dg[2][2];
#pragma unroll
    for (int c = 0; c < 2; ++c) {
        const int ch = 32 * c + l31;
        const float iv = a.f.invstd[0][ch], mu = a.f.mean[0][ch];
        const float c2p = a.chan_coef[64 + ch] * iv;
        const float c1p = a.chan_coef[ch] - c2p * mu;
        const __bf16 c1h = (__bf16)(-c1p);
        const __bf16 c1l = (__bf16)(-c1p - (float)c1h);
#pragma unroll
        for (int j = 0; j < 2; ++j)
#pragma unroll
            for (int i = 0; i < 8; ++i) {
                const int e = 8 * j + i;
                const int bs = (e & 3) + 8 * (e >> 2) + 4 * kh;
                float v = 0.f;
                if (bs < 20) v = sWf[(bs / 5) * 320 + (bs % 5) * 64 + ch];
                __bf16 q = (__bf16)v;
                if (bs == 24) q = c1h;
                if (bs == 25) q = c1l;
                wt[c][j][i] = q;
            }
#pragma unroll
        for (int gp = 0; gp < 2; ++gp)
#pragma unroll
            for (int i = 0; i < 8; ++i) dg[c][gp][i] = (__bf16)((16 * (2 * c + gp) + 8 * kh + i) == ch ? -c2p : 0.f);
    }
    const __bf16 one = (__bf16)1.f, zero = (__bf16)0.f;
    const __bf16* h = static_cast<const __bf16*>(a.f.h) + (size_t)n * HW * 64;
    __bf16* dh = static_cast<__bf16*>(a.dh) + (size_t)n * HW * 64;

    const int ngroup = (HW + 31) / 32;
    for (int grp = slice * 4 + wave; grp < ngroup; grp += 4 * S) {
        const int pbase = grp * 32;
        const bool live = pbase + l31 < HW;
        const int pl = live ? pbase + l31 : HW - 1;
        bf16x8 hb[4];
#pragma unroll
        for (int g = 0; g < 4; ++g) hb[g] = *reinterpret_cast<const bf16x8*>(h + (size_t)pl * 64 + (size_t)(g * 16 + kh * 8));
        float px[4], py[4];
#pragma unroll
        for (int b = 0; b < 4; ++b) { px[b] = a.f.pos_x[b][pl]; py[b] = a.f.pos_y[b][pl]; }
        f32x16 acc;
#pragma unroll
        for (int e = 0; e < 16; ++e) acc[e] = 0.f;
#pragma unroll
        for (int g = 0; g < 4; ++g) acc = __builtin_amdgcn_mfma_f32_32x32x16_bf16(wa[g], hb[g], acc, 0, 0, 0);
        if (split) {
#pragma unroll
            for (int g = 0; g < 4; ++g) acc = __builtin_amdgcn_mfma_f32_32x32x16_bf16(wal[g], hb[g], acc, 0, 0, 0);
        }
        bf16x8 db[2];
#pragma unroll
        for (int e = 0; e < 12; ++e) {
            const float d = __expf(acc[e] + ck0[e]) * ((cgx[e] * px[ebr[e]] + cgy[e] * py[ebr[e]]) - ccst[e]);
            db[e >> 3][e & 7] = (__bf16)d;
        }
        db[1][4] = kh == 0 ? one : zero;
        db[1][5] = kh == 0 ? one : zero;
        db[1][6] = zero; db[1][7] = zero;
        f32x16 o[2];
#pragma unroll
        for (int c = 0; c < 2; ++c) {
#pragma unroll
            for (int e = 0; e < 16; ++e) o[c][e] = 0.f;
#pragma unroll
            for (int j = 0; j < 2; ++j) o[c] = __builtin_amdgcn_mfma_f32_32x32x16_bf16(wt[c][j], db[j], o[c], 0, 0, 0);
#pragma unroll
            for (int gp = 0; gp < 2; ++gp) o[c] = __builtin_amdgcn_mfma_f32_32x32x16_bf16(dg[c][gp], hb[2 * c + gp], o[c], 0, 0, 0);
        }
        if (live) {
#pragma unroll
            for (int c = 0; c < 2; ++c)
#pragma unroll
                for (int q = 0; q < 4; ++q) {
                    const f32x4 v = {o[c][4 * q], o[c][4 * q + 1], o[c][4 * q + 2], o[c][4 * q + 3]};
                    *reinterpret_cast<bf16x4*>(dh + (size_t)(pbase + l31) * 64 + (size_t)(32 * c + 8 * q + 4 * kh)) = __builtin_convertvector(v, bf16x4);
                }
        }
    }
}

static int head_bwd_slices(int N, int HW)
{
    int S = (1024 + N - 1) / N;
    if (S > 16) S = 16;
    const int cap = ((HW + 31) / 32 + 3) / 4;
    if (S > cap) S = cap;
    return S < 1 ? 1 : S;
}
static bool head_bwd_mfma(const HeadArgs& f) { return f.act_bf16 && !lbc_opt_on(kOptHeadNoMfma); }

}

int lbc_head_fwd(const HeadArgs& a, hipStream_t s)
{
    LBC_REQUIRE(a.N > 0 && a.OH > 0 && a.OW > 0, "head_fwd: bad shape");
    LbcProfScope prof("head_fwd", 2.0 * a.N * a.OH * a.OW * 64.0 * 20, 4.0 * a.N * (double)a.OH * a.OW * 64, s);
    const bool no_mfma = lbc_opt_on(kOptHeadNoMfma);
    const int wsplit = a.act_bf16 ? 1 : 0;
    if (a.act_bf16 && !no_mfma) {
        HeadArgs b = a;
        b.nslice = 1; b.wsplit = wsplit;
        if (a.scratch) {
            b.nslice = (1024 + a.N - 1) / a.N;
            if (b.nslice > 16) b.nslice = 16;
            const int cap = ((a.OH * a.OW + 31) / 32 + 3) / 4;
            if (b.nslice > cap) b.nslice = cap;
            if (b.nslice < 1) b.nslice = 1;
        }
        hipLaunchKernelGGL(head_fwd_mfma_k, dim3((unsigned)a.N, (unsigned)b.nslice), dim3(256), 0, s, b);
        if (b.nslice > 1) hipLaunchKernelGGL(head_merge_k, dim3((unsigned)lbc_cdiv(a.N * 20, 256)), dim3(256), 0, s, b);
    }
    else if (a.act_bf16) { HeadArgs b = a; b.wsplit = wsplit; hipLaunchKernelGGL((head_fwd_k<__bf16>), dim3((unsigned)a.N, 4), dim3(256), 0, s, b); }
    else hipLaunchKernelGGL((head_fwd_k<float>), dim3((unsigned)a.N, 4), dim3(256), 0, s, a);
    int rc = lbc_check_launch("head_fwd");
    if (rc) return rc;
    if (a.pred_sel) {
        hipLaunchKernelGGL(select_branch_k, dim3((unsigned)lbc_cdiv(a.N * 10, 256)), dim3(256), 0, s, a.pred_all, a.cmd,
                           a.pred_sel, a.N);
        rc = lbc_check_launch("select_branch");
    }
    return rc;
}

int lbc_head_bwd_rows(const HeadArgs& f) { return head_bwd_mfma(f) ? f.N * head_bwd_slices(f.N, f.OH * f.OW) : f.N; }
int lbc_head_bwd_max_rows(int max_batch) { return max_batch + 1024; }

int lbc_head_bwd_reduce(const HeadBwdArgs& a0, hipStream_t s)
{
    HeadBwdArgs a = a0;
    a.f.wsplit = a.f.act_bf16 ? 1 : 0;
    LBC_REQUIRE(a.f.mean[0] == a.f.mean[1] && a.f.mean[0] == a.f.mean[2] && a.f.mean[0] == a.f.mean[3],
                "head backward requires training-mode (shared batch) statistics");
    LbcProfScope prof("head_bwd_reduce", 4.0 * a.f.N * a.f.OH * a.f.OW * 64.0 * 20, 4.0 * a.f.N * (double)a.f.OH * a.f.OW * 64, s);
    if (head_bwd_mfma(a.f)) {
        const int S = head_bwd_slices(a.f.N, a.f.OH * a.f.OW);
        hipLaunchKernelGGL(head_bwd_reduce_mfma_k, dim3((unsigned)a.f.N, (unsigned)S), dim3(256), 0, s, a, S);
        return lbc_check_launch("head_bwd_reduce");
    }
#define LBC_K(T, d) hipLaunchKernelGGL((head_bwd_reduce_k<T>), dim3((unsigned)a.f.N, 4), dim3(256), 0, s, a)
    LBC_DISPATCH_ACT(a.f.act_bf16, LBC_K, 0);
#undef LBC_K
    return lbc_check_launch("head_bwd_reduce");
}

int lbc_head_bwd_finalize(const HeadBwdFinalizeArgs& a, hipStream_t s)
{
    LbcProfScope prof("head_bwd_finalize", 0.0, 4.0 * (double)a.rows * 20 * 65, s);
    hipLaunchKernelGGL(head_bwd_finalize_k, dim3(1), dim3(256), 0, s, a);
    return lbc_check_launch("head_bwd_finalize");
}

int lbc_head_bwd_apply(const HeadBwdArgs& a0, hipStream_t s)
{
    HeadBwdArgs a = a0;
    a.f.wsplit = a.f.act_bf16 ? 1 : 0;
    const int HW = a.f.OH * a.f.OW;
    LbcProfScope prof("head_bwd_apply", 4.0 * a.f.N * (double)HW * 64.0 * 20, 8.0 * a.f.N * (double)HW * 64, s);
    if (head_bwd_mfma(a.f)) {
        const int S = head_bwd_slices(a.f.N, HW);
        hipLaunchKernelGGL(head_bwd_apply_mfma_k, dim3((unsigned)a.f.N, (unsigned)S), dim3(256), 0, s, a, S);
        return lbc_check_launch("head_bwd_apply");
    }
#define LBC_K(T, d) hipLaunchKernelGGL((head_bwd_apply_k<T>), dim3((unsigned)a.f.N, (unsigned)lbc_cdiv(HW, TP)), dim3(256), 0, s, a)
    LBC_DISPATCH_ACT(a.f.act_bf16, LBC_K, 0);
#undef LBC_K
    return lbc_check_launch("head_bwd_apply");
}
```

### learningbycheating_amd/csrc/lbc_kernels.hpp

```cpp
#pragma once
#include "lbc_common.hpp"

constexpr int kLbcFinalizeRows = 1024;
struct BnFinalizeArgs {
    const float* partial;
    int rows, C;
    long long count;
    const float* nsum; int n_local;
    const float* gamma;
    const float* beta;
    float* running_mean;
    float* running_var;
    long long* num_batches_tracked;
    float* more_running_mean[3]; float* more_running_var[3]; long long* more_num_batches_tracked[3];
    float momentum, eps;
    int train;
    float* scale;
    float* shift;
    float* save_mean;
    float* save_invstd;
};
struct BnEvalItem {
    const float* gamma; const float* beta; const float* running_mean; const float* running_var;
    float* scale; float* shift; float* mean; float* invstd;
    int C;
};
struct BnEvalArgs {
    static const int kMax = 48;
    BnEvalItem item[kMax];
    int count;
    float eps;
};
int lbc_bn_eval_prep(const BnEvalArgs& a, hipStream_t s);
int lbc_partial_reduce(const float* in, int rows, int cols, float* out, int out_rows, hipStream_t s, float* copy_lo = nullptr,
                       float* copy_hi = nullptr, float tail = -1.f);
int lbc_bn_finalize(const BnFinalizeArgs& a, hipStream_t s);

struct BnApplyArgs {
    const void* x; void* y;
    long long pixels; int C;
    const float* scale; const float* shift;
    const void* resid;
    const float* rscale;
    const float* rshift;
    int relu;
    int act_bf16;
    int fold, rfold;
    BnFinalizeArgs fin, rfin;
};
int lbc_bn_apply(const BnApplyArgs& a, hipStream_t s);
bool lbc_bn_fold_ok(int rows, int C);
int lbc_bn_fold_max_rows(int C);

struct ChanReduceArgs {
    const void* x;
    const void* dz;
    const void* mask;
    const float* mask_scale;
    const float* mask_shift;
    void* g_out;
    const float* mean;
    const float* invstd;
    float* partial;
    long long pixels; int C;
    long long pix_per_block;
    int act_bf16;
    int max_rows;
};
int lbc_chan_reduce_rows(long long pixels, int C, int max_rows = 0);
int lbc_chan_reduce(ChanReduceArgs a, int op, hipStream_t s);

struct BnBwdFinalizeArgs {
    const float* partial; int rows, C; long long count;
    const float* nsum; int n_local;
    const float* gamma; const float* mean; const float* invstd;
    int train;
    float* dgamma; float* dbeta;
    float* coefA; float* coefB; float* coefD;
};
int lbc_bn_bwd_finalize(const BnBwdFinalizeArgs& a, hipStream_t s);

struct BnBwdApplyArgs {
    const void* g; const void* mask; const void* x;
    const float* coefA; const float* coefB; const float* coefD;
    const float* mean; const float* invstd;
    void* dx;
    long long pixels; int C, Cout;
    int accum;
    int act_bf16;
    int fold;
    BnBwdFinalizeArgs fin;
};
int lbc_bn_bwd_apply(const BnBwdApplyArgs& a, hipStream_t s);

int lbc_copy_f32(const float* src, float* dst, long long n, hipStream_t s);
int lbc_concat_velocity(const void* t, const float* vel, void* h, int N, int hw, int Ct, int Cv, int act_bf16, hipStream_t s);

struct NormConst { float mean[8]; float stdv[8]; int enabled; };
int lbc_prep_input(const float* img_nchw, void* xp, int xp_bf16, int N, int C, int H, int W, const NormConst& nc, hipStream_t s);
int lbc_prep_input_u8(const unsigned char* img_nhwc, void* xp, int xp_bf16, int N, int C, int H, int W, const NormConst& nc, hipStream_t s);
struct StemArgs {
    const void* xp;
    int xp_bf16;
    const float* w;
    void* y;
    float* stats;
    int N, H, W, Cin;
    int act_bf16;
    int bf16;
};
int lbc_stem_rows(const StemArgs& a);
int lbc_stem_fwd(const StemArgs& a, hipStream_t s);
struct StemWgradArgs {
    const void* xp; int xp_bf16; const void* dy; float* partial;
    int N, H, W, Cin, nsplit;
    int act_bf16;
    int bf16;
    const void* bn_y;
    const float* bn_coefA; const float* bn_coefB; const float* bn_coefD; const float* bn_mean; const float* bn_invstd;
};
bool lbc_stem_wgrad_fuses_bn_bwd(int Cin, int bf16);
int lbc_stem_wgrad_split(int N, int H, int W, int Cin, int bf16);
int lbc_stem_wgrad(const StemWgradArgs& a, hipStream_t s);

struct PoolFwdArgs {
    const void* y;
    const float* scale; const float* shift;
    void* p;
    unsigned char* idx;
    int N, H, W, C;
    int act_bf16;
};
int lbc_bn_relu_maxpool_fwd(const PoolFwdArgs& a, hipStream_t s);
struct PoolBwdArgs {
    const void* dp;
    const unsigned char* idx;
    const void* y;
    const float* scale; const float* shift;
    const float* mean; const float* invstd;
    void* g;
    float* partial;
    int N, H, W, C;
    long long pix_per_block;
    int act_bf16;
};
int lbc_pool_bwd_rows(int N, int H, int W, int C);
int lbc_maxpool_relu_bwd_reduce(PoolBwdArgs a, hipStream_t s);

struct HeadArgs {
    const void* h;
    int act_bf16;
    const float* mean[4];
    const float* invstd[4];
    const float* gamma[4];
    const float* beta[4];
    const float* w[4];
    const float* bias[4];
    const float* cmd;
    const float* pos_x[4];
    const float* pos_y[4];
    float* pred_all;
    float* pred_sel;
    float* rowstat;
    int N, OH, OW;
    float* scratch;
    int nslice;
    int wsplit;
};
int lbc_head_fwd(const HeadArgs& a, hipStream_t s);
struct HeadBwdArgs {
    HeadArgs f;
    const float* d_all;
    const float* d_sel;
    float* s_partial;
    void* dh;
    const float* chan_coef;
};
int lbc_head_bwd_rows(const HeadArgs& f);
int lbc_head_bwd_max_rows(int max_batch);
int lbc_head_bwd_reduce(const HeadBwdArgs& a, hipStream_t s);
struct HeadBwdFinalizeArgs {
    const float* s_partial; int rows; long long count;
    const float* nsum; int n_local;
    const float* gamma[4]; const float* beta[4]; const float* w[4];
    const float* mean; const float* invstd;
    float* dgamma[4]; float* dbeta[4]; float* dw[4]; float* dbias[4];
    float* chan_coef;
    int coef_only;
};
int lbc_head_bwd_finalize(const HeadBwdFinalizeArgs& a, hipStream_t s);
int lbc_head_bwd_apply(const HeadBwdArgs& a, hipStream_t s);

enum { kAugBlur = 0, kAugNoise = 1, kAugCoarseDropout = 2, kAugDropout = 3, kAugAdd = 4, kAugMultiply = 5, kAugContrast = 6 };
struct WarpParams {
    double im[6];
    int y0, x0;
};
int lbc_warp_crop_u8(const unsigned char* src, unsigned char* dst, const WarpParams* params_dev, int N, int SH, int SW, int C, int H, int W, hipStream_t s);
struct AugParams {
    int order[8];
    int n_ops;
    int blur_pos;
    unsigned seed;
    float blur_sigma;
    float noise_scale; int noise_pc;
    float cd_p; int cd_h, cd_w, cd_pc;
    float do_p; int do_pc;
    float add_v[3], mul_v[3], con_a[3];
};
int lbc_crop_u8(const unsigned char* src, unsigned char* dst, int N, int SH, int SW, int C, int y0, int x0, int H, int W, hipStream_t s);
int lbc_augment_u8(unsigned char* img, const AugParams* params_dev, float* tmp, int N, int H, int W, int any_blur, hipStream_t s);

int lbc_replay_cdf_launch(const float* w, int n, double* cdf, long long* bad_count, hipStream_t s);
int lbc_replay_sample_launch(const double* cdf, int n, unsigned seed, unsigned long long step, int B, int* idx, hipStream_t s);
int lbc_replay_gather_launch(const unsigned char* src, long long row_bytes, const int* idx, int B, int reps, unsigned char* dst, hipStream_t s);
int lbc_replay_scatter_launch(const unsigned char* src, long long row_bytes, const int* slot, int M, unsigned char* dst, hipStream_t s);
int lbc_replay_meta_launch(const float* speed, const int* cmd, const int* idx, int B, int reps, float* speed_out, float* onehot_out, hipStream_t s);
int lbc_replay_writeback_launch(const float* w_batch, const int* idx, int B, int reps, int n, float* new_w, hipStream_t s);

struct LossArgs {
    const float* pred;
    const float* target;
    float* loss_per_sample;
    float* dpred;
    int N, R;
    float grad_scale;
    float w, h, fov, world_y, fixed_offset, pixels_per_meter, crop_size;
};
int lbc_loss_phase1(const LossArgs& a, hipStream_t s);
int lbc_loss_phase0(const LossArgs& a, hipStream_t s);
int lbc_loss_l1(const LossArgs& a, float target_scale, float target_shift, hipStream_t s);
int lbc_phase2_weight_launch(const LossArgs& a, hipStream_t s);

struct AdamChunk { float* p; const float* g; float* m; float* v; int n; int pad; };
int lbc_adam_launch(const AdamChunk* chunks_dev, int nchunks, double lr, double beta1, double beta2, double eps,
                    double weight_decay, int step, hipStream_t s);
long long lbc_adam_profile_elems_get();
struct lbc_adam_state;
int lbc_adam_guarded_launch(const AdamChunk* chunks_dev, int nchunks, double lr, double beta1, double beta2, double eps,
                            double weight_decay, lbc_adam_state* state_dev, hipStream_t s);
struct lbc_adam_clip_state;
int lbc_adam_clipped_launch(const AdamChunk* chunks_dev, int nchunks, double lr, double beta1, double beta2, double eps,
                            double weight_decay, double max_norm, lbc_adam_clip_state* state_dev, hipStream_t s);
void lbc_adam_norm_pass(const AdamChunk* chunks_dev, int nchunks, lbc_adam_clip_state* state_dev, double* partial, hipStream_t s);
struct lbc_adam_recipe;
struct lbc_adam_recipe_state;
int lbc_adam_recipe_launch(const AdamChunk* chunks_dev, int nchunks, const lbc_adam_recipe* recipe, float* const* ema_dev,
                           lbc_adam_recipe_state* state_dev, hipStream_t s);
int lbc_grad_accumulate_launch(const float* g, float* acc, long long n, int first, hipStream_t s);
struct lbc_waypoint_metrics_desc;
int lbc_waypoint_metrics_launch(const lbc_waypoint_metrics_desc* d, const float* pred, const float* target, const float* command_onehot,
                                const float* loss, int N, void* state, hipStream_t s);
```

### learningbycheating_amd/csrc/pool.hip

```cpp
#include "lbc_common.hpp"
#include "lbc_act.hpp"
#include "lbc_kernels.hpp"

namespace {

__device__ __forceinline__ unsigned xcd_major_block()
{
    const unsigned nwg = gridDim.x, b = blockIdx.x;
    const unsigned xcd = b & 7u, q = nwg >> 3, rr = nwg & 7u;
    return (xcd < rr ? xcd * (q + 1) : rr * (q + 1) + (xcd - rr) * q) + (b >> 3);
}

template <typename T, typename IDX>
__global__ __launch_bounds__(256) void bn_relu_maxpool_fwd_k(PoolFwdArgs a)
{
    constexpr int V = Act<T>::kVec;
    using vec = typename Act<T>::vec;
    using PV = ParamVec<V>;
    const T* y = static_cast<const T*>(a.y);
    T* pout = static_cast<T*>(a.p);
    const int OH = a.H / 2, OW = a.W / 2;
    const int cvn = a.C / V;
    const IDX total = (IDX)((long long)a.N * OH * OW * cvn);
    const IDX stride = (IDX)gridDim.x * (IDX)blockDim.x;
    const IDX span = (total + (IDX)gridDim.x - 1) / (IDX)gridDim.x;
    const IDX i0 = (IDX)xcd_major_block() * span;
    const IDX i1 = i0 + span < total ? i0 + span : total;
    (void)stride;
    for (IDX i = i0 + (IDX)threadIdx.x; i < i1; i += (IDX)blockDim.x) {
        IDX t = i;
        const int cg = (int)(t % (IDX)cvn); t /= (IDX)cvn;
        const int ox = (int)(t % (IDX)OW); t /= (IDX)OW;
        const int oy = (int)(t % (IDX)OH);
        const int n = (int)(t / (IDX)OH);
        const int c = cg * V;
        const vec sc = PV::ld(a.scale + c), sh = PV::ld(a.shift + c);
        vec best = PV::splat(-INFINITY);
        int bi[V];
#pragma unroll
        for (int e = 0; e < V; ++e) bi[e] = 0;
        typename Act<T>::raw raw[9];
        bool ok[9];
#pragma unroll
        for (int r = 0; r < 3; ++r) {
            const int iy = 2 * oy - 1 + r;
            const bool oky = (unsigned)iy < (unsigned)a.H;
            const int cy = oky ? iy : oy * 2;
#pragma unroll
            for (int s = 0; s < 3; ++s) {
                const int ix = 2 * ox - 1 + s;
                const bool okx = (unsigned)ix < (unsigned)a.W;
                const int cx = okx ? ix : ox * 2;
                ok[r * 3 + s] = oky && okx;
                raw[r * 3 + s] = Act<T>::ldr(y + ((size_t)(n * a.H + cy) * a.W + (size_t)cx) * a.C + c);
            }
        }
#pragma unroll
        for (int tap = 0; tap < 9; ++tap) {
            vec v = Act<T>::cvt(raw[tap]);
            v = v * sc + sh;
#pragma unroll
            for (int e = 0; e < V; ++e) {
                const float z = ok[tap] ? fmaxf(v[e], 0.f) : -INFINITY;
                if (z > best[e]) { best[e] = z; bi[e] = tap; }
            }
        }
        Act<T>::stv(pout + i * V, best);
        if (a.idx) {
#pragma unroll
            for (int q = 0; q < V / 4; ++q) {
                uchar4 u;
                u.x = (unsigned char)bi[4 * q]; u.y = (unsigned char)bi[4 * q + 1]; u.z = (unsigned char)bi[4 * q + 2]; u.w = (unsigned char)bi[4 * q + 3];
                reinterpret_cast<uchar4*>(a.idx)[i * (V / 4) + q] = u;
            }
        }
    }
}

template <typename T, typename IDX>
__global__ __launch_bounds__(256) void maxpool_relu_bwd_reduce_k(PoolBwdArgs a)
{
    constexpr int V = Act<T>::kVec;
    using vec = typename Act<T>::vec;
    using PV = ParamVec<V>;
    __shared__ __attribute__((aligned(16))) float red[2 * 256 * V];
    const T* dp = static_cast<const T*>(a.dp);
    const T* y = static_cast<const T*>(a.y);
    T* gout = static_cast<T*>(a.g);
    const int OH = a.H / 2, OW = a.W / 2;
    const int cvn = a.C / V;
    const int rl = 256 / cvn;
    const int cg = threadIdx.x % cvn;
    const int pl = threadIdx.x / cvn;
    const int c = cg * V;
    vec s1 = PV::splat(0.f), s2 = s1;
    if (pl < rl) {
        const vec sc = PV::ld(a.scale + c), sh = PV::ld(a.shift + c);
        const vec mean = PV::ld(a.mean + c), inv = PV::ld(a.invstd + c);
        const long long pixels = (long long)a.N * a.H * a.W;
        const long long p0 = (long long)xcd_major_block() * a.pix_per_block;
        long long p1 = p0 + a.pix_per_block;
        if (p1 > pixels) p1 = pixels;
        for (long long p = p0 + pl; p < p1; p += rl) {
            const IDX pi = (IDX)p;
            const int x = (int)(pi % (IDX)a.W);
            const IDX t = pi / (IDX)a.W;
            const int yy = (int)(t % (IDX)a.H);
            const int n = (int)(t / (IDX)a.H);
            vec g = PV::splat(0.f);
            const int oy0 = yy >> 1, oy1 = (yy + 1) >> 1;
            const int ox0 = x >> 1, ox1 = (x + 1) >> 1;
            const bool rok = oy1 != oy0 && oy1 < OH, cok = ox1 != ox0 && ox1 < OW;
            const int oyw[2] = {oy0, rok ? oy1 : oy0}, oxw[2] = {ox0, cok ? ox1 : ox0};
            typename Act<T>::raw draw[4];
            uchar4 uraw[4][V / 4];
#pragma unroll
            for (int wv = 0; wv < 4; ++wv) {
                const size_t o = ((size_t)(n * OH + oyw[wv >> 1]) * OW + (size_t)oxw[wv & 1]) * cvn + cg;
                draw[wv] = Act<T>::ldr(dp + o * V);
#pragma unroll
                for (int q = 0; q < V / 4; ++q) uraw[wv][q] = reinterpret_cast<const uchar4*>(a.idx)[o * (V / 4) + q];
            }
            const typename Act<T>::raw yraw = Act<T>::ldr(y + (p * cvn + cg) * V);
#pragma unroll
            for (int wv = 0; wv < 4; ++wv) {
                const bool okw = ((wv >> 1) == 0 || rok) && ((wv & 1) == 0 || cok);
                const int tap = okw ? (yy - (2 * oyw[wv >> 1] - 1)) * 3 + (x - (2 * oxw[wv & 1] - 1)) : 255;
                const vec d = Act<T>::cvt(draw[wv]);
#pragma unroll
                for (int q = 0; q < V / 4; ++q) {
                    const uchar4 u = uraw[wv][q];
                    if (u.x == tap) g[4 * q] += d[4 * q];
                    if (u.y == tap) g[4 * q + 1] += d[4 * q + 1];
                    if (u.z == tap) g[4 * q + 2] += d[4 * q + 2];
                    if (u.w == tap) g[4 * q + 3] += d[4 * q + 3];
                }
            }
            const vec v = Act<T>::cvt(yraw);
            const vec z = v * sc + sh;
#pragma unroll
            for (int e = 0; e < V; ++e) g[e] = z[e] > 0.f ? g[e] : 0.f;
            Act<T>::stv(gout + (p * cvn + cg) * V, g);
            s1 += g;
            s2 += g * (v - mean) * inv;
        }
    }
    PV::st(red + threadIdx.x * V, s1);
    PV::st(red + (256 + threadIdx.x) * V, s2);
    __syncthreads();
    if (threadIdx.x < cvn) {
        vec t1 = PV::splat(0.f), t2 = t1;
        for (int k = 0; k < rl; ++k) {
            t1 += PV::ld(red + (k * cvn + threadIdx.x) * V);
            t2 += PV::ld(red + (256 + k * cvn + threadIdx.x) * V);
        }
        float* dst = a.partial + (size_t)blockIdx.x * 2 * a.C;
        PV::st(dst + c, t1);
        PV::st(dst + a.C + c, t2);
    }
}

}

int lbc_bn_relu_maxpool_fwd(const PoolFwdArgs& a, hipStream_t s)
{
    LBC_REQUIRE(a.C % 8 == 0 && a.H % 2 == 0 && a.W % 2 == 0, "maxpool: bad shape");
    const long long total = (long long)a.N * (a.H / 2) * (a.W / 2) * (a.C / 4);
    long long blocks = (total / (a.act_bf16 ? 2 : 1) + 255) / 256;
    if (blocks > 8192) blocks = 8192;
    LbcProfScope prof("bn_relu_maxpool_fwd", 0.0, (a.act_bf16 ? 2.0 : 4.0) * total * 4 * (4.0 + 1.0) + total * 4.0, s);
    const bool small = total + blocks * 256 < (1ll << 31);
#define LBC_K(T, g)                                                                                                          \
    do {                                                                                                                     \
        if (small) hipLaunchKernelGGL((bn_relu_maxpool_fwd_k<T, unsigned>), dim3((unsigned)(g)), dim3(256), 0, s, a);        \
        else       hipLaunchKernelGGL((bn_relu_maxpool_fwd_k<T, long long>), dim3((unsigned)(g)), dim3(256), 0, s, a);       \
    } while (0)
    LBC_DISPATCH_ACT(a.act_bf16, LBC_K, blocks);
#undef LBC_K
    return lbc_check_launch("bn_relu_maxpool_fwd");
}

int lbc_pool_bwd_rows(int N, int H, int W, int C) { return lbc_chan_reduce_rows((long long)N * H * W, C); }

int lbc_maxpool_relu_bwd_reduce(PoolBwdArgs a, hipStream_t s)
{
    LBC_REQUIRE(a.C % 8 == 0 && a.C / 4 <= 256, "maxpool_bwd: bad C");
    const long long pixels = (long long)a.N * a.H * a.W;
    const int rows = lbc_pool_bwd_rows(a.N, a.H, a.W, a.C);
    a.pix_per_block = (pixels + rows - 1) / rows;
    LbcProfScope prof("maxpool_relu_bwd_reduce", 0.0, (a.act_bf16 ? 2.0 : 4.0) * (double)pixels * a.C * (2.0 + 0.25) + (double)pixels * a.C * 0.25, s);
    const bool small = pixels < (1ll << 31);
#define LBC_K(T, g)                                                                                                              \
    do {                                                                                                                         \
        if (small) hipLaunchKernelGGL((maxpool_relu_bwd_reduce_k<T, unsigned>), dim3((unsigned)(g)), dim3(256), 0, s, a);        \
        else       hipLaunchKernelGGL((maxpool_relu_bwd_reduce_k<T, long long>), dim3((unsigned)(g)), dim3(256), 0, s, a);       \
    } while (0)
    LBC_DISPATCH_ACT(a.act_bf16, LBC_K, rows);
#undef LBC_K
    return lbc_check_launch("maxpool_relu_bwd_reduce");
}
```

Before: 17090 images/sec.

## Precompute head BN-folded weights once, prefetch head tiles, specialize maxpool backward

A new small kernel folds the head BatchNorm into the 1x1 projection once per forward and stores it in a workspace buffer. The forward and backward MFMA head kernels now load that buffer instead of each block recomputing the fold. The head loops software-prefetch the next activation group and hoist the pos_x/pos_y loads. The maxpool backward is templated on pixel parity so it gathers only the windows that can contain each pixel, with a remapped lane-to-pixel assignment. The finalize reduction is also unrolled by 8. The backward kernels now rely on the fold buffer left by the forward, which adds an ordering dependency between them.

```diff
diff --git a/learningbycheating_amd/csrc/c_api_ops.cpp b/learningbycheating_amd/csrc/c_api_ops.cpp
--- a/learningbycheating_amd/csrc/c_api_ops.cpp
+++ b/learningbycheating_amd/csrc/c_api_ops.cpp
@@ -127,13 +127,15 @@
 }
 
 namespace {
-struct HeadWs { float* rowstat; float* s_partial; float* partial2; float* coef; float* scratch; };
+struct HeadWs { float* rowstat; float* s_partial; float* partial2; float* coef; float* scratch; float* fold; };
 HeadWs head_ws(float* w, int N)
 {
     HeadWs h;
     h.rowstat = w;
     h.s_partial = h.rowstat + up64((size_t)N * 40);
     h.partial2 = h.s_partial + up64((size_t)lbc_head_bwd_max_rows(N) * 20 * 65);
+    static_assert(kHeadFoldFloats <= 20 * 65, "head workspace: the folded projection must fit one partial row");
+    h.fold = h.s_partial + (size_t)(lbc_head_bwd_max_rows(N) - 1) * 20 * 65;
     h.coef = h.partial2 + up64((size_t)8 * 20 * 65);
     h.scratch = h.coef + up64((size_t)3 * 64);
     return h;
@@ -162,7 +164,7 @@
     HeadArgs ha;
     head_args(d, ha);
     const HeadWs ws = head_ws(workspace, d->N);
-    ha.pred_all = pred_all; ha.pred_sel = pred_sel; ha.rowstat = ws.rowstat; ha.scratch = ws.scratch;
+    ha.pred_all = pred_all; ha.pred_sel = pred_sel; ha.rowstat = ws.rowstat; ha.scratch = ws.scratch; ha.fold = ws.fold;
     return lbc_head_fwd(ha, (hipStream_t)stream);
 }
 
@@ -177,7 +179,7 @@
     HeadBwdArgs hb;
     memset(&hb, 0, sizeof(hb));
     head_args(d, hb.f);
-    hb.f.pred_all = const_cast<float*>(pred_all); hb.f.rowstat = ws.rowstat;
+    hb.f.pred_all = const_cast<float*>(pred_all); hb.f.rowstat = ws.rowstat; hb.f.fold = ws.fold;
     hb.d_all = d_all; hb.d_sel = d_sel; hb.s_partial = ws.s_partial; hb.dh = dh; hb.chan_coef = ws.coef;
     LBC_TRY(lbc_head_bwd_reduce(hb, s));
     HeadBwdFinalizeArgs hf;
diff --git a/learningbycheating_amd/csrc/engine.cpp b/learningbycheating_amd/csrc/engine.cpp
--- a/learningbycheating_amd/csrc/engine.cpp
+++ b/learningbycheating_amd/csrc/engine.cpp
@@ -144,6 +144,7 @@
     }
     head_stats_ = alloc(2 * 64);
     head_coef_ = alloc(3 * 64);
+    head_fold_ = alloc(kHeadFoldFloats);
     head_partial_ = alloc(std::max((size_t)lbc_head_bwd_max_rows((int)NB) * 20 * 65, NB * 16 * 20 * 4));
     pred_all_ = alloc(NB * 40);
     rowstat_ = alloc(NB * 40);
@@ -599,6 +600,7 @@
     ha.pred_all = W(pred_all_); ha.pred_sel = pred_sel; ha.rowstat = W(rowstat_);
     ha.N = N; ha.OH = HH_; ha.OW = HW_; ha.act_bf16 = act_bf16_;
     ha.scratch = W(head_partial_);
+    ha.fold = W(head_fold_);
     LBC_TRY(lbc_head_fwd(ha, s));
     return lbc_copy_f32(W(pred_all_), pred_all, 40 * N, s);
 }
@@ -894,7 +896,7 @@
             ha.pos_x[b] = P(head_px_[b]); ha.pos_y[b] = P(head_py_[b]);
         }
         ha.cmd = W(cmd_); ha.pred_all = W(pred_all_); ha.rowstat = W(rowstat_);
-        ha.N = N; ha.OH = HH_; ha.OW = HW_; ha.act_bf16 = act_bf16_;
+        ha.N = N; ha.OH = HH_; ha.OW = HW_; ha.act_bf16 = act_bf16_; ha.fold = W(head_fold_);
         hb.d_all = d_all; hb.d_sel = d_sel; hb.s_partial = W(head_partial_); hb.dh = E; hb.chan_coef = W(head_coef_);
         LBC_TRY(lbc_head_bwd_reduce(hb, s));
         HeadBwdFinalizeArgs hf;
diff --git a/learningbycheating_amd/csrc/engine.hpp b/learningbycheating_amd/csrc/engine.hpp
--- a/learningbycheating_amd/csrc/engine.hpp
+++ b/learningbycheating_amd/csrc/engine.hpp
@@ -151,7 +151,7 @@
     int HH_ = 0, HW_ = 0;
 
     size_t xp_ = 0, y0_ = 0, p0_ = 0, idx_ = 0, hcat_ = 0, cmd_ = 0;
-    size_t partial_ = 0, partial2_ = 0, wg_partial_ = 0, head_partial_ = 0, head_coef_ = 0, head_stats_ = 0;
+    size_t partial_ = 0, partial2_ = 0, wg_partial_ = 0, head_partial_ = 0, head_coef_ = 0, head_stats_ = 0, head_fold_ = 0;
     size_t pred_all_ = 0, rowstat_ = 0;
     size_t gD_ = 0, gE_ = 0, gF_ = 0, gG_ = 0, g0_ = 0;
     size_t partial_floats_ = 0, partial2_floats_ = 0;
diff --git a/learningbycheating_amd/csrc/head.hip b/learningbycheating_amd/csrc/head.hip
--- a/learningbycheating_amd/csrc/head.hip
+++ b/learningbycheating_amd/csrc/head.hip
@@ -36,13 +36,18 @@
     }
 }
 
-__device__ __forceinline__ void fold_branch(const HeadArgs& a, int b, float* sW , float* sB , int tid, int nthr)
-{
-    const float* mean = a.mean[b];
-    const float* inv = a.invstd[b];
+struct HeadBranch { const float* mean; const float* inv; const float* gamma; const float* beta; const float* w; const float* bias; };
+__device__ __forceinline__ HeadBranch head_branch(const HeadArgs& a, int b)
+{
+    return HeadBranch{a.mean[b], a.invstd[b], a.gamma[b], a.beta[b], a.w[b], a.bias[b]};
+}
+__device__ __forceinline__ void fold_branch(const HeadArgs& a, const HeadBranch& br, float* sW , float* sB , int tid, int nthr)
+{
+    const float* mean = br.mean;
+    const float* inv = br.inv;
     for (int idx = tid; idx < 320; idx += nthr) {
         const int c = idx & 63;
-        const float wf = a.w[b][idx] * a.gamma[b][c] * inv[c];
+        const float wf = br.w[idx] * br.gamma[c] * inv[c];
         float v = wf;
         if (a.act_bf16) {
             const float hi = (float)(__bf16)wf;
@@ -51,9 +56,9 @@
         sW[idx] = v;
     }
     if (tid < 5) {
-        float t = a.bias[b][tid];
+        float t = br.bias[tid];
         for (int c = 0; c < 64; ++c)
-            t += a.w[b][tid * 64 + c] * (a.beta[b][c] - a.gamma[b][c] * mean[c] * inv[c]);
+            t += br.w[tid * 64 + c] * (br.beta[c] - br.gamma[c] * mean[c] * inv[c]);
         sB[tid] = t;
     }
 }
@@ -68,7 +73,7 @@
     const int tid = threadIdx.x, lane = tid & 63, wave = tid >> 6;
     const int n = blockIdx.x, b = blockIdx.y;
     const int HW = a.OH * a.OW;
-    fold_branch(a, b, sW, sB, tid, 256);
+    fold_branch(a, head_branch(a, b), sW, sB, tid, 256);
     __syncthreads();
 
     SoftAcc st[5];
@@ -129,6 +134,33 @@
         a.pred_all[o2 + 1] = t.sy / t.l;
         if (a.rowstat) { a.rowstat[o2] = t.m; a.rowstat[o2 + 1] = t.l; }
     }
+}
+
+__global__ __launch_bounds__(256) void head_fold_k(HeadArgs a)
+{
+    __shared__ float sP[4 * 64 + 320 + 8];
+    const int tid = threadIdx.x, b = blockIdx.x;
+    const HeadBranch g = head_branch(a, b);
+    if (tid < 64) { sP[tid] = g.mean[tid]; sP[64 + tid] = g.inv[tid]; sP[128 + tid] = g.gamma[tid]; sP[192 + tid] = g.beta[tid]; }
+    for (int idx = tid; idx < 320; idx += 256) sP[256 + idx] = g.w[idx];
+    if (tid < 5) sP[576 + tid] = g.bias[tid];
+    __syncthreads();
+    const HeadBranch l = {sP, sP + 64, sP + 128, sP + 192, sP + 256, sP + 576};
+    fold_branch(a, l, a.fold + b * 320, a.fold + 4 * 320 + b * 5, tid, 256);
+}
+
+__device__ __forceinline__ void load_fold(const float* fold, float* sWf, float* sBf, int tid)
+{
+#pragma unroll
+    for (int j = 0; j < 5; ++j) sWf[tid + 256 * j] = fold[tid + 256 * j];
+    if (tid < 20) sBf[(tid / 5) * 8 + tid % 5] = fold[4 * 320 + tid];
+}
+
+__device__ __forceinline__ void load_group(const __bf16* h, int HW, int grp, int l31, int kh, bf16x8 (&af)[4])
+{
+    const int pl = grp * 32 + l31 < HW ? grp * 32 + l31 : HW - 1;
+#pragma unroll
+    for (int g = 0; g < 4; ++g) af[g] = *reinterpret_cast<const bf16x8*>(h + (size_t)pl * 64 + (size_t)(g * 16 + kh * 8));
 }
 
 __global__ __launch_bounds__(256) void head_fwd_mfma_k(HeadArgs a)
@@ -141,7 +173,7 @@
     const int n = blockIdx.x;
     const int HW = a.OH * a.OW;
     const int S = a.nslice, slice = blockIdx.y;
-    for (int b = 0; b < 4; ++b) fold_branch(a, b, sWf + b * 320, sBf + b * 8, tid, 256);
+    load_fold(a.fold, sWf, sBf, tid);
     __syncthreads();
     const bool colok = l31 < 20;
     const int cb = colok ? l31 / 5 : 0, cs = colok ? l31 - 5 * cb : 0;
@@ -162,15 +194,24 @@
 
     SoftAcc st; st.m = -INFINITY; st.l = 0.f; st.sx = 0.f; st.sy = 0.f;
     const int ngroup = (HW + 31) / 32;
+    bf16x8 an[4];
+    if (slice * 4 + wave < ngroup) load_group(h, HW, slice * 4 + wave, l31, kh, an);
     for (int grp = slice * 4 + wave; grp < ngroup; grp += 4 * S) {
         const int pbase = grp * 32;
-        const int pl = pbase + l31 < HW ? pbase + l31 : HW - 1;
+        bf16x8 af[4];
+#pragma unroll
+        for (int g = 0; g < 4; ++g) af[g] = an[g];
+        float px[16], py[16];
+#pragma unroll
+        for (int e = 0; e < 16; ++e) {
+            const int p = pbase + (e & 3) + 8 * (e >> 2) + 4 * kh;
+            const int pc = p < HW ? p : HW - 1;
+            px[e] = posx[pc]; py[e] = posy[pc];
+        }
+        load_group(h, HW, grp + 4 * S < ngroup ? grp + 4 * S : grp, l31, kh, an);
         f32x16 acc;
 #pragma unroll
         for (int e = 0; e < 16; ++e) acc[e] = 0.f;
-        bf16x8 af[4];
-#pragma unroll
-        for (int g = 0; g < 4; ++g) af[g] = *reinterpret_cast<const bf16x8*>(h + (size_t)pl * 64 + (size_t)(g * 16 + kh * 8));
 #pragma unroll
         for (int g = 0; g < 4; ++g) acc = __builtin_amdgcn_mfma_f32_32x32x16_bf16(af[g], wb[g], acc, 0, 0, 0);
         if (split) {
@@ -190,10 +231,8 @@
             st.l *= f; st.sx *= f; st.sy *= f; st.m = M;
 #pragma unroll
             for (int e = 0; e < 16; ++e) {
-                const int p = pbase + (e & 3) + 8 * (e >> 2) + 4 * kh;
-                const int pc = p < HW ? p : HW - 1;
                 const float w = __expf(acc[e] - M);
-                st.l += w; st.sx += w * posx[pc]; st.sy += w * posy[pc];
+                st.l += w; st.sx += w * px[e]; st.sy += w * py[e];
             }
         }
     }
@@ -277,7 +316,7 @@
     const int tid = threadIdx.x, lane = tid & 63, wave = tid >> 6;
     const int n = blockIdx.x, b = blockIdx.y;
     const int HW = a.f.OH * a.f.OW;
-    fold_branch(a.f, b, sW, sB, tid, 256);
+    fold_branch(a.f, head_branch(a.f, b), sW, sB, tid, 256);
     if (tid < 5) {
         float gx, gy;
         row_grad(a, n, b, tid, gx, gy);
@@ -358,7 +397,13 @@
     const int tid = threadIdx.x;
     for (int idx = tid; idx < 20 * 65; idx += 256) {
         double t = 0.0;
-        for (int r = 0; r < a.rows; ++r) t += (double)a.s_partial[(size_t)r * (20 * 65) + idx];
+        for (int r0 = 0; r0 < a.rows; r0 += 8) {
+            float v[8];
+#pragma unroll
+            for (int j = 0; j < 8; ++j) v[j] = a.s_partial[(size_t)(r0 + j < a.rows ? r0 + j : a.rows - 1) * (20 * 65) + idx];
+#pragma unroll
+            for (int j = 0; j < 8; ++j) t = r0 + j < a.rows ? t + (double)v[j] : t;
+        }
         sS[idx] = (float)t;
     }
     __syncthreads();
@@ -410,7 +455,7 @@
     const int tid = threadIdx.x;
     const int n = blockIdx.x, tile = blockIdx.y;
     const int HW = a.f.OH * a.f.OW;
-    for (int b = 0; b < 4; ++b) fold_branch(a.f, b, sW + b * 320, sB + b * 8, tid, 256);
+    for (int b = 0; b < 4; ++b) fold_branch(a.f, head_branch(a.f, b), sW + b * 320, sB + b * 8, tid, 256);
     if (tid < 20) {
         const int b = tid / 5, s = tid - b * 5;
         float gx, gy;
@@ -499,7 +544,7 @@
     const int l31 = lane & 31, kh = lane >> 5, G1 = (lane >> 4) & 1, t16 = lane & 15;
     const int n = blockIdx.x, slice = blockIdx.y;
     const int HW = a.f.OH * a.f.OW;
-    for (int b = 0; b < 4; ++b) fold_branch(a.f, b, sWf + b * 320, sBf + b * 8, tid, 256);
+    load_fold(a.f.fold, sWf, sBf, tid);
     __syncthreads();
     head_row_consts(a, n, sBf, sRow, tid);
     __syncthreads();
@@ -529,12 +574,21 @@
         for (int e = 0; e < 16; ++e) accH[c][e] = 0.f;
     float s0 = 0.f, s0r = 0.f;
     const int ngroup = (HW + 31) / 32;
+    bf16x8 an[4];
+    if (slice * 4 + wave < ngroup) load_group(h, HW, slice * 4 + wave, l31, kh, an);
     for (int grp = slice * 4 + wave; grp < ngroup; grp += 4 * S) {
         const int pbase = grp * 32;
-        const int pl = pbase + l31 < HW ? pbase + l31 : HW - 1;
         bf16x8 af[4];
 #pragma unroll
-        for (int g = 0; g < 4; ++g) af[g] = *reinterpret_cast<const bf16x8*>(h + (size_t)pl * 64 + (size_t)(g * 16 + kh * 8));
+        for (int g = 0; g < 4; ++g) af[g] = an[g];
+        float px[16], py[16];
+#pragma unroll
+        for (int e = 0; e < 16; ++e) {
+            const int p = pbase + (e & 3) + 8 * (e >> 2) + 4 * kh;
+            const int pc = p < HW ? p : HW - 1;
+            px[e] = posx[pc]; py[e] = posy[pc];
+        }
+        load_group(h, HW, grp + 4 * S < ngroup ? grp + 4 * S : grp, l31, kh, an);
 #pragma unroll
         for (int g = 0; g < 4; ++g) *reinterpret_cast<bf16x8*>(&tile[l31 * kHTS + g * 16 + kh * 8]) = af[g];
         f32x16 acc;
@@ -551,7 +605,7 @@
         for (int e = 0; e < 16; ++e) {
             const int p = pbase + (e & 3) + 8 * (e >> 2) + 4 * kh;
             float d = 0.f;
-            if (p < HW && colok) d = __expf(acc[e] + k0) * ((gx * posx[p] + gy * posy[p]) - cst);
+            if (p < HW && colok) d = __expf(acc[e] + k0) * ((gx * px[e] + gy * py[e]) - cst);
             const __bf16 dr = (__bf16)d;
             db[e >> 3][e & 7] = dr;
             s0 += d;
@@ -597,7 +651,7 @@
     const int l31 = lane & 31, kh = lane >> 5;
     const int n = blockIdx.x, slice = blockIdx.y;
     const int HW = a.f.OH * a.f.OW;
-    for (int b = 0; b < 4; ++b) fold_branch(a.f, b, sWf + b * 320, sBf + b * 8, tid, 256);
+    load_fold(a.f.fold, sWf, sBf, tid);
     __syncthreads();
     head_row_consts(a, n, sBf, sRow, tid);
     __syncthreads();
@@ -657,16 +711,19 @@
     __bf16* dh = static_cast<__bf16*>(a.dh) + (size_t)n * HW * 64;
 
     const int ngroup = (HW + 31) / 32;
+    bf16x8 hn[4];
+    if (slice * 4 + wave < ngroup) load_group(h, HW, slice * 4 + wave, l31, kh, hn);
     for (int grp = slice * 4 + wave; grp < ngroup; grp += 4 * S) {
         const int pbase = grp * 32;
         const bool live = pbase + l31 < HW;
         const int pl = live ? pbase + l31 : HW - 1;
         bf16x8 hb[4];
 #pragma unroll
-        for (int g = 0; g < 4; ++g) hb[g] = *reinterpret_cast<const bf16x8*>(h + (size_t)pl * 64 + (size_t)(g * 16 + kh * 8));
+        for (int g = 0; g < 4; ++g) hb[g] = hn[g];
         float px[4], py[4];
 #pragma unroll
         for (int b = 0; b < 4; ++b) { px[b] = a.f.pos_x[b][pl]; py[b] = a.f.pos_y[b][pl]; }
+        load_group(h, HW, grp + 4 * S < ngroup ? grp + 4 * S : grp, l31, kh, hn);
         f32x16 acc;
 #pragma unroll
         for (int e = 0; e < 16; ++e) acc[e] = 0.f;
@@ -707,7 +764,7 @@
     }
 }
 
-static int head_bwd_slices(int N, int HW)
+static int head_slices(int N, int HW)
 {
     int S = (1024 + N - 1) / N;
     if (S > 16) S = 16;
@@ -715,6 +772,7 @@
     if (S > cap) S = cap;
     return S < 1 ? 1 : S;
 }
+static int head_bwd_slices(int N, int HW) { return head_slices(N, HW); }
 static bool head_bwd_mfma(const HeadArgs& f) { return f.act_bf16 && !lbc_opt_on(kOptHeadNoMfma); }
 
 }
@@ -722,19 +780,17 @@
 int lbc_head_fwd(const HeadArgs& a, hipStream_t s)
 {
     LBC_REQUIRE(a.N > 0 && a.OH > 0 && a.OW > 0, "head_fwd: bad shape");
-    LbcProfScope prof("head_fwd", 2.0 * a.N * a.OH * a.OW * 64.0 * 20, 4.0 * a.N * (double)a.OH * a.OW * 64, s);
+    LbcProfScope prof("head_fwd", 2.0 * a.N * a.OH * a.OW * 64.0 * 20, (a.act_bf16 ? 2.0 : 4.0) * a.N * (double)a.OH * a.OW * 64, s);
     const bool no_mfma = lbc_opt_on(kOptHeadNoMfma);
     const int wsplit = a.act_bf16 ? 1 : 0;
     if (a.act_bf16 && !no_mfma) {
         HeadArgs b = a;
         b.nslice = 1; b.wsplit = wsplit;
         if (a.scratch) {
-            b.nslice = (1024 + a.N - 1) / a.N;
-            if (b.nslice > 16) b.nslice = 16;
-            const int cap = ((a.OH * a.OW + 31) / 32 + 3) / 4;
-            if (b.nslice > cap) b.nslice = cap;
-            if (b.nslice < 1) b.nslice = 1;
-        }
+            b.nslice = head_slices(a.N, a.OH * a.OW);
+        }
+        LBC_REQUIRE(a.fold, "head_fwd: the bf16 head needs HeadArgs::fold");
+        hipLaunchKernelGGL(head_fold_k, dim3(4), dim3(256), 0, s, b);
         hipLaunchKernelGGL(head_fwd_mfma_k, dim3((unsigned)a.N, (unsigned)b.nslice), dim3(256), 0, s, b);
         if (b.nslice > 1) hipLaunchKernelGGL(head_merge_k, dim3((unsigned)lbc_cdiv(a.N * 20, 256)), dim3(256), 0, s, b);
     }
@@ -759,8 +815,9 @@
     a.f.wsplit = a.f.act_bf16 ? 1 : 0;
     LBC_REQUIRE(a.f.mean[0] == a.f.mean[1] && a.f.mean[0] == a.f.mean[2] && a.f.mean[0] == a.f.mean[3],
                 "head backward requires training-mode (shared batch) statistics");
-    LbcProfScope prof("head_bwd_reduce", 4.0 * a.f.N * a.f.OH * a.f.OW * 64.0 * 20, 4.0 * a.f.N * (double)a.f.OH * a.f.OW * 64, s);
+    LbcProfScope prof("head_bwd_reduce", 4.0 * a.f.N * a.f.OH * a.f.OW * 64.0 * 20, (a.f.act_bf16 ? 2.0 : 4.0) * a.f.N * (double)a.f.OH * a.f.OW * 64, s);
     if (head_bwd_mfma(a.f)) {
+        LBC_REQUIRE(a.f.fold, "head_bwd_reduce: the bf16 head needs HeadArgs::fold as the forward left it");
         const int S = head_bwd_slices(a.f.N, a.f.OH * a.f.OW);
         hipLaunchKernelGGL(head_bwd_reduce_mfma_k, dim3((unsigned)a.f.N, (unsigned)S), dim3(256), 0, s, a, S);
         return lbc_check_launch("head_bwd_reduce");
@@ -783,8 +840,9 @@
     HeadBwdArgs a = a0;
     a.f.wsplit = a.f.act_bf16 ? 1 : 0;
     const int HW = a.f.OH * a.f.OW;
-    LbcProfScope prof("head_bwd_apply", 4.0 * a.f.N * (double)HW * 64.0 * 20, 8.0 * a.f.N * (double)HW * 64, s);
+    LbcProfScope prof("head_bwd_apply", 4.0 * a.f.N * (double)HW * 64.0 * 20, (a.f.act_bf16 ? 4.0 : 8.0) * a.f.N * (double)HW * 64, s);
     if (head_bwd_mfma(a.f)) {
+        LBC_REQUIRE(a.f.fold, "head_bwd_apply: the bf16 head needs HeadArgs::fold as the forward left it");
         const int S = head_bwd_slices(a.f.N, HW);
         hipLaunchKernelGGL(head_bwd_apply_mfma_k, dim3((unsigned)a.f.N, (unsigned)S), dim3(256), 0, s, a, S);
         return lbc_check_launch("head_bwd_apply");
diff --git a/learningbycheating_amd/csrc/lbc_kernels.hpp b/learningbycheating_amd/csrc/lbc_kernels.hpp
--- a/learningbycheating_amd/csrc/lbc_kernels.hpp
+++ b/learningbycheating_amd/csrc/lbc_kernels.hpp
@@ -166,7 +166,9 @@
     float* scratch;
     int nslice;
     int wsplit;
-};
+    float* fold;
+};
+constexpr int kHeadFoldFloats = 4 * 320 + 20;
 int lbc_head_fwd(const HeadArgs& a, hipStream_t s);
 struct HeadBwdArgs {
     HeadArgs f;
diff --git a/learningbycheating_amd/csrc/pool.hip b/learningbycheating_amd/csrc/pool.hip
--- a/learningbycheating_amd/csrc/pool.hip
+++ b/learningbycheating_amd/csrc/pool.hip
@@ -77,6 +77,47 @@
     }
 }
 
+template <typename T, bool YO, bool XO>
+__device__ __forceinline__ typename Act<T>::vec pool_bwd_gather(const T* dp, const unsigned char* idx, int n, int yy, int x, int OH, int OW,
+                                                                int cvn, int cg)
+{
+    constexpr int V = Act<T>::kVec;
+    using vec = typename Act<T>::vec;
+    constexpr int NY = YO ? 2 : 1, NX = XO ? 2 : 1;
+    const int oy0 = yy >> 1, ox0 = x >> 1;
+    const bool rok = YO && oy0 + 1 < OH, cok = XO && ox0 + 1 < OW;
+    const int oyw[2] = {oy0, rok ? oy0 + 1 : oy0}, oxw[2] = {ox0, cok ? ox0 + 1 : ox0};
+    typename Act<T>::raw draw[NY * NX];
+    uchar4 uraw[NY * NX][V / 4];
+#pragma unroll
+    for (int wy = 0; wy < NY; ++wy)
+#pragma unroll
+        for (int wx = 0; wx < NX; ++wx) {
+            const size_t o = ((size_t)(n * OH + oyw[wy]) * OW + (size_t)oxw[wx]) * cvn + cg;
+            draw[wy * NX + wx] = Act<T>::ldr(dp + o * V);
+#pragma unroll
+            for (int q = 0; q < V / 4; ++q) uraw[wy * NX + wx][q] = reinterpret_cast<const uchar4*>(idx)[o * (V / 4) + q];
+        }
+    vec g = ParamVec<V>::splat(0.f);
+#pragma unroll
+    for (int wy = 0; wy < NY; ++wy)
+#pragma unroll
+        for (int wx = 0; wx < NX; ++wx) {
+            const bool okw = (wy == 0 || rok) && (wx == 0 || cok);
+            const int tap = okw ? (yy - (2 * oyw[wy] - 1)) * 3 + (x - (2 * oxw[wx] - 1)) : 255;
+            const vec d = Act<T>::cvt(draw[wy * NX + wx]);
+#pragma unroll
+            for (int q = 0; q < V / 4; ++q) {
+                const uchar4 u = uraw[wy * NX + wx][q];
+                if (u.x == tap) g[4 * q] += d[4 * q];
+                if (u.y == tap) g[4 * q + 1] += d[4 * q + 1];
+                if (u.z == tap) g[4 * q + 2] += d[4 * q + 2];
+                if (u.w == tap) g[4 * q + 3] += d[4 * q + 3];
+            }
+        }
+    return g;
+}
+
 template <typename T, typename IDX>
 __global__ __launch_bounds__(256) void maxpool_relu_bwd_reduce_k(PoolBwdArgs a)
 {
@@ -91,7 +132,8 @@
     const int cvn = a.C / V;
     const int rl = 256 / cvn;
     const int cg = threadIdx.x % cvn;
-    const int pl = threadIdx.x / cvn;
+    const int slot = threadIdx.x / cvn;
+    const int pl = (rl & 1) || slot >= rl ? slot : (slot < rl / 2 ? 2 * slot : 2 * (slot - rl / 2) + 1);
     const int c = cg * V;
     vec s1 = PV::splat(0.f), s2 = s1;
     if (pl < rl) {
@@ -107,34 +149,14 @@
             const IDX t = pi / (IDX)a.W;
             const int yy = (int)(t % (IDX)a.H);
             const int n = (int)(t / (IDX)a.H);
-            vec g = PV::splat(0.f);
-            const int oy0 = yy >> 1, oy1 = (yy + 1) >> 1;
-            const int ox0 = x >> 1, ox1 = (x + 1) >> 1;
-            const bool rok = oy1 != oy0 && oy1 < OH, cok = ox1 != ox0 && ox1 < OW;
-            const int oyw[2] = {oy0, rok ? oy1 : oy0}, oxw[2] = {ox0, cok ? ox1 : ox0};
-            typename Act<T>::raw draw[4];
-            uchar4 uraw[4][V / 4];
-#pragma unroll
-            for (int wv = 0; wv < 4; ++wv) {
-                const size_t o = ((size_t)(n * OH + oyw[wv >> 1]) * OW + (size_t)oxw[wv & 1]) * cvn + cg;
-                draw[wv] = Act<T>::ldr(dp + o * V);
-#pragma unroll
-                for (int q = 0; q < V / 4; ++q) uraw[wv][q] = reinterpret_cast<const uchar4*>(a.idx)[o * (V / 4) + q];
-            }
             const typename Act<T>::raw yraw = Act<T>::ldr(y + (p * cvn + cg) * V);
-#pragma unroll
-            for (int wv = 0; wv < 4; ++wv) {
-                const bool okw = ((wv >> 1) == 0 || rok) && ((wv & 1) == 0 || cok);
-                const int tap = okw ? (yy - (2 * oyw[wv >> 1] - 1)) * 3 + (x - (2 * oxw[wv & 1] - 1)) : 255;
-                const vec d = Act<T>::cvt(draw[wv]);
-#pragma unroll
-                for (int q = 0; q < V / 4; ++q) {
-                    const uchar4 u = uraw[wv][q];
-                    if (u.x == tap) g[4 * q] += d[4 * q];
-                    if (u.y == tap) g[4 * q + 1] += d[4 * q + 1];
-                    if (u.z == tap) g[4 * q + 2] += d[4 * q + 2];
-                    if (u.w == tap) g[4 * q + 3] += d[4 * q + 3];
-                }
+            vec g;
+            if (yy & 1) {
+                if (x & 1) g = pool_bwd_gather<T, true, true>(dp, a.idx, n, yy, x, OH, OW, cvn, cg);
+                else       g = pool_bwd_gather<T, true, false>(dp, a.idx, n, yy, x, OH, OW, cvn, cg);
+            } else {
+                if (x & 1) g = pool_bwd_gather<T, false, true>(dp, a.idx, n, yy, x, OH, OW, cvn, cg);
+                else       g = pool_bwd_gather<T, false, false>(dp, a.idx, n, yy, x, OH, OW, cvn, cg);
             }
             const vec v = Act<T>::cvt(yraw);
             const vec z = v * sc + sh;
@@ -145,8 +167,9 @@
             s2 += g * (v - mean) * inv;
         }
     }
-    PV::st(red + threadIdx.x * V, s1);
-    PV::st(red + (256 + threadIdx.x) * V, s2);
+    const int rslot = pl < rl ? pl * cvn + cg : (int)threadIdx.x;
+    PV::st(red + rslot * V, s1);
+    PV::st(red + (256 + rslot) * V, s2);
     __syncthreads();
     if (threadIdx.x < cvn) {
         vec t1 = PV::splat(0.f), t2 = t1;
```

Result: no change. 17200 images/sec (median of 6 runs) (+0.7%).
